# shadygm/Lichtfeld-Densification-Plugin

Hardware: AMD Instinct MI355X
Metric: triangulated points/sec + pairs/sec, MipNeRF360 garden @fast, 1/2/4/8 GPU (higher is better)
Workload: dtype f32 (+f64 Sampson/DLT solve)

## Files before the change

### include/lfd_densify.h

```cpp
#ifndef LFD_DENSIFY_H
#define LFD_DENSIFY_H

#include <stdint.h>

#ifdef __cplusplus
extern "C" {
#endif

#define LFD_ABI_VERSION 9
#define LFD_MAX_SLOTS 16

enum lfd_status {
    LFD_OK = 0,
    LFD_ERR_INVALID = 1,
    LFD_ERR_HIP = 2,
    LFD_ERR_CAPACITY = 3,
    LFD_ERR_STATE = 4
};

typedef struct lfd_context lfd_context;

typedef struct lfd_params {
    double sampson_thresh;
    float certainty_thresh;
    float sample_cap;
    float reproj_thresh;
    float min_parallax_deg;
    int32_t no_filter;
    int32_t flags;
} lfd_params;

#define LFD_FLAG_EXACT_COLOUR 1

typedef struct lfd_batch {
    int32_t n_refs;
    int32_t k;
    int32_t H, W;
    int32_t w_match, h_match;
    int32_t warp_channels;
    int32_t reserved;
    const int32_t* ref_cam;
    const int32_t* n_slots;
    const int32_t* nbr_cam;
    const float* const* cert;
    const float* const* warp;
    const uint8_t* const* image;
    const uint8_t* const* mask_a;
    const uint8_t* const* mask_b;
    const float* axis_x;
    const float* axis_y;
    const float* fundamental;
} lfd_batch;

typedef struct lfd_points {
    float* xyz;
    float* rgb;
    float* err;
    int32_t* cell;
    uint8_t* slot;
    int64_t capacity;
} lfd_points;

int lfd_abi_version(void);
int lfd_create(int device_index, void* hip_stream, lfd_context** out);
void lfd_destroy(lfd_context* ctx);
int lfd_set_stream(lfd_context* ctx, void* hip_stream);
int lfd_reload_env(lfd_context* ctx);
int lfd_kernel_timing(lfd_context* ctx, int32_t n_launches);
int lfd_kernel_timing_read(lfd_context* ctx, float* ms, int32_t capacity, int32_t* n_out);
const char* lfd_last_error(const lfd_context* ctx);
int lfd_struct_layout(int32_t* out, int32_t capacity);
const char* lfd_struct_fields(void);

int lfd_upload_cameras(lfd_context* ctx, int32_t n, const float* K, const float* R, const float* t,
                       const float* P, const float* C, const int32_t* wh);

int lfd_prepare_batch(lfd_context* ctx, const lfd_batch* batch, const lfd_params* params);

int lfd_aggregate(lfd_context* ctx, const lfd_batch* batch, const lfd_params* params,
                  float* best_cert, uint8_t* best_slot);

int lfd_triangulate_dense(lfd_context* ctx, const lfd_batch* batch, const lfd_params* params,
                          const lfd_points* out, int64_t* ref_offsets, int32_t* seg_counts);

int lfd_triangulate_dense_ply(lfd_context* ctx, const lfd_batch* batch, const lfd_params* params, uint8_t* records, int64_t capacity,
                              int64_t* ref_offsets, int32_t* seg_counts, int32_t* cell, uint8_t* slot);

typedef struct lfd_tile_segment { int32_t offset; int32_t count; } lfd_tile_segment;
#define LFD_FLAG_TILE_SEGMENTS 2
int lfd_dense_tiles_per_ref(int32_t H, int32_t W);
int lfd_triangulate_dense_segments(lfd_context* ctx, const lfd_batch* batch, const lfd_params* params, const lfd_points* out,
                                   int64_t* ref_counts, int32_t* seg_counts, lfd_tile_segment* table);
int lfd_triangulate_dense_ply_segments(lfd_context* ctx, const lfd_batch* batch, const lfd_params* params, uint8_t* records, int64_t capacity,
                                       int64_t* ref_counts, int32_t* seg_counts, lfd_tile_segment* table);
int lfd_order_segments(lfd_context* ctx, int32_t n_refs, int32_t H, int32_t W, const lfd_tile_segment* table, const lfd_points* src,
                       const lfd_points* dst, int64_t* ref_offsets);
int lfd_pack_ply_segments(lfd_context* ctx, int32_t n_refs, int32_t H, int32_t W, const lfd_tile_segment* table, const float* xyz,
                          const float* rgb, int64_t capacity, uint8_t* out, int64_t* ref_offsets);
int lfd_pack_points3d_segments(lfd_context* ctx, int32_t n_refs, int32_t H, int32_t W, const lfd_tile_segment* table, const float* xyz,
                               const float* rgb, const float* err, int64_t capacity, uint64_t id_base, uint8_t* out, int64_t* ref_offsets);

int lfd_triangulate_indexed(lfd_context* ctx, const lfd_batch* batch, const lfd_params* params,
                            const int64_t* sel_idx, const int64_t* sel_offsets, const lfd_points* out,
                            int64_t* ref_offsets, int32_t* seg_counts, int32_t* seg_order);

int lfd_triangulate_sampled(lfd_context* ctx, const lfd_batch* batch, const lfd_params* params, int32_t M, float cap,
                            int32_t border, int32_t tiles, float s_override, const lfd_points* out, int64_t* ref_offsets,
                            int32_t* seg_counts, int32_t* seg_order, int32_t* sel_info, int64_t* sel_cells);

int lfd_triangulate_sampled_multi(lfd_context* ctx, const lfd_batch* batch, const lfd_params* params, int32_t M, float cap,
                                  int32_t border, int32_t tiles, const uint32_t* seeds, const lfd_points* out,
                                  int64_t* ref_offsets, int32_t* seg_counts, int32_t* seg_order, int32_t* sel_info,
                                  int64_t* sel_cells);

int lfd_triangulate_sampled_chain(lfd_context* ctx, const lfd_batch* batch, const lfd_params* params, int32_t M, float cap,
                                  int32_t border, int32_t tiles, const float* s_overrides, const lfd_points* out,
                                  int64_t* ref_offsets, int32_t* seg_counts, int32_t* seg_order, int32_t* sel_info,
                                  int64_t* sel_cells);

int lfd_rng_seed(lfd_context* ctx, uint32_t seed);
int lfd_rng_get_state(lfd_context* ctx, uint32_t* key624_host, int32_t* pos_host);
int lfd_rng_set_state(lfd_context* ctx, const uint32_t* key624_host, int32_t pos);
#define LFD_RNG_CHECKPOINTS 4
int lfd_rng_checkpoint(lfd_context* ctx, int32_t place);
int lfd_rng_rollback(lfd_context* ctx, int32_t place);
int lfd_select_samples(lfd_context* ctx, const float* best_cert, int32_t H, int32_t W, int32_t M, float cap,
                       int32_t border, int32_t tiles, float s_override, int64_t* sel_out, int64_t capacity,
                       int32_t* n_sel_host, int32_t* status_host);

int lfd_select_top_m(lfd_context* ctx, const float* best_cert, int32_t H, int32_t W, int32_t M, float cap,
                     int64_t* sel_out, int64_t capacity, int32_t* n_sel_host, int32_t* status_host);

int lfd_pack_ply(lfd_context* ctx, const float* xyz, const float* rgb, int64_t n, uint8_t* out);
int lfd_pack_ply_normals(lfd_context* ctx, const float* xyz, const float* normals, const float* rgb, int64_t n, uint8_t* out);
int lfd_pack_points3d(lfd_context* ctx, const float* xyz, const float* rgb, const float* err, int64_t n,
                      uint64_t id_base, uint8_t* out);
int lfd_quantise_rgb(lfd_context* ctx, const float* rgb, int64_t n, uint8_t* out);

int lfd_voxel_downsample(lfd_context* ctx, const float* xyz, const float* rgb, int64_t n, double voxel_size,
                         float* xyz_out, float* rgb_out, int64_t* n_out_host);

int lfd_local_corr(lfd_context* ctx, const float* A, const float* Bf, const float* warp, int32_t B, int32_t N, int32_t C, int32_t K,
                   int32_t H1, int32_t W1, const int64_t* a_strides, const int64_t* bf_strides, float* out);
int lfd_local_corr_host(lfd_context* ctx, const float* A, const float* Bf, const float* warp, int32_t B, int32_t N, int32_t C, int32_t K,
                        int32_t H1, int32_t W1, const int64_t* a_strides, const int64_t* bf_strides, float* out);

int lfd_refiner_block(lfd_context* ctx, const void* x, int32_t x_is_f32, int32_t B, int32_t C, int32_t H, int32_t W,
                      const float* dw_w, const float* scale, const float* shift, const float* pw_wT, const float* pw_b, uint16_t* out);
int lfd_refiner_block_host(lfd_context* ctx, const void* x, int32_t x_is_f32, int32_t B, int32_t C, int32_t H, int32_t W,
                           const float* dw_w, const float* scale, const float* shift, const float* pw_wT, const float* pw_b, uint16_t* out);

int lfd_refiner_head(lfd_context* ctx, const void* z, int32_t z_is_f32, int32_t B, int32_t C, int32_t H, int32_t W, const float* head_w,
                     const float* head_b, const float* prev_warp, const int64_t* prev_warp_strides, const float* prev_conf,
                     const int64_t* prev_conf_strides, int32_t prev_dim, float refine_init, float* warp, float* conf);
int lfd_refiner_head_host(lfd_context* ctx, const void* z, int32_t z_is_f32, int32_t B, int32_t C, int32_t H, int32_t W, const float* head_w,
                          const float* head_b, const float* prev_warp, const int64_t* prev_warp_strides, const float* prev_conf,
                          const int64_t* prev_conf_strides, int32_t prev_dim, float refine_init, float* warp, float* conf);

int lfd_cycle_gate(lfd_context* ctx, int32_t n_pairs, const float* const* cert, const float* const* warp_ab, const float* const* warp_ba, int32_t H,
                   int32_t W, int32_t warp_channels, int32_t Hb, int32_t Wb, const float* axis_x, const float* axis_y, int32_t w_match,
                   int32_t h_match, float certainty_thresh, float cycle_thresh_px, float* const* cert_out, float* const* err_out,
                   int32_t* rejected);
int lfd_cycle_gate_host(lfd_context* ctx, int32_t n_pairs, const float* const* cert, const float* const* warp_ab, const float* const* warp_ba,
                        int32_t H, int32_t W, int32_t warp_channels, int32_t Hb, int32_t Wb, const float* axis_x, const float* axis_y,
                        int32_t w_match, int32_t h_match, float certainty_thresh, float cycle_thresh_px, float* const* cert_out,
                        float* const* err_out, int32_t* rejected);

// ... 171 lines not shown
```

### lichtfeld-densification-plugin_amd/core/hip_backend.py

```python
from __future__ import annotations

import ctypes as C
import threading
import dataclasses
import os
from typing import List, Optional, Sequence, Tuple

import numpy as np
import torch

from .types import CameraRecord, DensePipelineConfig

LFD_MAX_SLOTS = 16
LFD_ABI_VERSION = 9
LFD_CONSENSUS_CAP = 8
LFD_FLAG_EXACT_COLOUR = 1
LFD_FLAG_TILE_SEGMENTS = 2
_LIB_NAME = "liblfd_densify.so"
_PKG_DIR = os.path.dirname(os.path.dirname(os.path.abspath(__file__)))


class HipBackendError(RuntimeError):
    """Raised for any non-zero status of the HIP library (message from ``lfd_last_error``)."""

# ... 53 lines not shown
    _fields_ = [("xyz", C.c_void_p), ("rgb", C.c_void_p), ("err", C.c_void_p), ("cell", C.c_void_p),
                ("slot", C.c_void_p), ("capacity", C.c_int64)]


class lfd_tile_segment(C.Structure):
    _fields_ = [("offset", C.c_int32), ("count", C.c_int32)]


class lfd_copy_segment(C.Structure):
    _fields_ = [("src_offset", C.c_int64), ("dst_offset", C.c_int64), ("nbytes", C.c_int64)]


ABI_STRUCTS = (lfd_params, lfd_batch, lfd_points, lfd_tile_segment, lfd_copy_segment)


def check_struct_layout(lib, structs=ABI_STRUCTS) -> None:
    lib.lfd_struct_layout.argtypes = [C.POINTER(C.c_int32), C.c_int32]
    lib.lfd_struct_layout.restype = C.c_int
    n = int(lib.lfd_struct_layout(None, 0))
    table = (C.c_int32 * n)()
    lib.lfd_struct_layout(table, n)
    lib.lfd_struct_fields.restype = C.c_char_p
    names = dict(part.split(":") for part in lib.lfd_struct_fields().decode().split(";"))
    vals, at = list(table), 0
    for cls in structs:
        theirs = names.get(cls.__name__, "").split(",")
        if [name for name, *_ in cls._fields_] != theirs:
            raise HipBackendError(f"ctypes mirror of {cls.__name__} lists the fields {[name for name, *_ in cls._fields_]}, the library's header has "
                                  f"{theirs} (include/lfd_densify.h and core/hip_backend.py disagree)")
        if at + 2 > len(vals):
            raise HipBackendError(f"lfd_struct_layout ends before {cls.__name__}: the library is older than this binding")
        size, n_fields = vals[at], vals[at + 1]
        offsets = list(zip(vals[at + 2:at + 2 + 2 * n_fields:2], vals[at + 3:at + 2 + 2 * n_fields:2]))
        at += 2 + 2 * n_fields
        mine = [(name, getattr(cls, name).offset, getattr(cls, name).size) for name, *_ in cls._fields_]
        if C.sizeof(cls) != size or [(o, z) for _n, o, z in mine] != offsets:
            raise HipBackendError(f"ctypes mirror of {cls.__name__} does not match the library's layout: here sizeof {C.sizeof(cls)} with offsets "
                                  f"(name, offset, size) {mine}, the library has sizeof {size} with (offset, size) {offsets} (include/lfd_densify.h and core/hip_backend.py disagree)")
    if at != len(vals):
        raise HipBackendError("lfd_struct_layout reports structures this binding does not mirror")


_lib = None


def library_path() -> str:
    return os.environ.get("LFD_DENSIFY_LIB") or os.path.join(_PKG_DIR, _LIB_NAME)


def load_library() -> C.CDLL:
    global _lib
    if _lib is not None:
        return _lib
    path = library_path()
    if not os.path.exists(path):
        raise HipBackendError(
            f"{path} not found: build it with `python {os.path.join(_PKG_DIR, 'csrc', 'build.py')}` "
            "(hipcc, --offload-arch=gfx950). There is no CPU fallback for the dense-initialisation path.")
    lib = C.CDLL(path)
    ctxp = C.c_void_p
    lib.lfd_abi_version.restype = C.c_int
    if int(lib.lfd_abi_version()) != LFD_ABI_VERSION:
        raise HipBackendError(f"{path} implements ABI {int(lib.lfd_abi_version())}, this binding ABI {LFD_ABI_VERSION}: rebuild the library "
                              f"(python {os.path.join(_PKG_DIR, 'csrc', 'build.py')})")
    check_struct_layout(lib)
    lib.lfd_create.argtypes = [C.c_int, C.c_void_p, C.POINTER(ctxp)]
    lib.lfd_destroy.argtypes = [ctxp]
    lib.lfd_destroy.restype = None
    lib.lfd_set_stream.argtypes = [ctxp, C.c_void_p]
    lib.lfd_reload_env.argtypes = [ctxp]
    lib.lfd_kernel_timing.argtypes = [ctxp, C.c_int32]
    lib.lfd_kernel_timing_read.argtypes = [ctxp, C.POINTER(C.c_float), C.c_int32, C.POINTER(C.c_int32)]
    lib.lfd_last_error.argtypes = [ctxp]
    lib.lfd_last_error.restype = C.c_char_p
    fptr = C.POINTER(C.c_float)
    lib.lfd_upload_cameras.argtypes = [ctxp, C.c_int32, fptr, fptr, fptr, fptr, fptr, C.POINTER(C.c_int32)]
    lib.lfd_prepare_batch.argtypes = [ctxp, C.POINTER(lfd_batch), C.POINTER(lfd_params)]
    lib.lfd_aggregate.argtypes = [ctxp, C.POINTER(lfd_batch), C.POINTER(lfd_params), C.c_void_p, C.c_void_p]
    lib.lfd_triangulate_dense.argtypes = [ctxp, C.POINTER(lfd_batch), C.POINTER(lfd_params), C.POINTER(lfd_points),
                                          C.c_void_p, C.c_void_p]
    lib.lfd_triangulate_dense_ply.argtypes = [ctxp, C.POINTER(lfd_batch), C.POINTER(lfd_params), C.c_void_p, C.c_int64, C.c_void_p, C.c_void_p,
                                              C.c_void_p, C.c_void_p]
    lib.lfd_dense_tiles_per_ref.argtypes = [C.c_int32, C.c_int32]
    lib.lfd_triangulate_dense_segments.argtypes = [ctxp, C.POINTER(lfd_batch), C.POINTER(lfd_params), C.POINTER(lfd_points),
                                                   C.c_void_p, C.c_void_p, C.c_void_p]
    lib.lfd_triangulate_dense_ply_segments.argtypes = [ctxp, C.POINTER(lfd_batch), C.POINTER(lfd_params), C.c_void_p, C.c_int64, C.c_void_p, C.c_void_p, C.c_void_p]
    lib.lfd_order_segments.argtypes = [ctxp, C.c_int32, C.c_int32, C.c_int32, C.c_void_p, C.POINTER(lfd_points), C.POINTER(lfd_points), C.c_void_p]
    lib.lfd_pack_ply_segments.argtypes = [ctxp, C.c_int32, C.c_int32, C.c_int32, C.c_void_p, C.c_void_p, C.c_void_p, C.c_int64, C.c_void_p, C.c_void_p]
    lib.lfd_pack_points3d_segments.argtypes = [ctxp, C.c_int32, C.c_int32, C.c_int32, C.c_void_p, C.c_void_p, C.c_void_p, C.c_void_p, C.c_int64,
                                               C.c_uint64, C.c_void_p, C.c_void_p]
    lib.lfd_triangulate_indexed.argtypes = [ctxp, C.POINTER(lfd_batch), C.POINTER(lfd_params), C.c_void_p,
                                            C.POINTER(C.c_int64), C.POINTER(lfd_points), C.c_void_p, C.c_void_p,
                                            C.c_void_p]
    lib.lfd_triangulate_sampled.argtypes = [ctxp, C.POINTER(lfd_batch), C.POINTER(lfd_params), C.c_int32, C.c_float, C.c_int32,
                                            C.c_int32, C.c_float, C.POINTER(lfd_points), C.c_void_p, C.c_void_p, C.c_void_p,
                                            C.c_void_p, C.c_void_p]
    lib.lfd_triangulate_sampled_multi.argtypes = [ctxp, C.POINTER(lfd_batch), C.POINTER(lfd_params), C.c_int32, C.c_float, C.c_int32,
                                                  C.c_int32, C.POINTER(C.c_uint32), C.POINTER(lfd_points), C.c_void_p, C.c_void_p, C.c_void_p,
                                                  C.c_void_p, C.c_void_p]
    lib.lfd_triangulate_sampled_chain.argtypes = [ctxp, C.POINTER(lfd_batch), C.POINTER(lfd_params), C.c_int32, C.c_float, C.c_int32,
                                                  C.c_int32, C.POINTER(C.c_float), C.POINTER(lfd_points), C.c_void_p, C.c_void_p, C.c_void_p,
                                                  C.c_void_p, C.c_void_p]
    lib.lfd_select_top_m.argtypes = [ctxp, C.c_void_p, C.c_int32, C.c_int32, C.c_int32, C.c_float, C.c_void_p, C.c_int64,
                                     C.POINTER(C.c_int32), C.POINTER(C.c_int32)]
    lib.lfd_pack_ply.argtypes = [ctxp, C.c_void_p, C.c_void_p, C.c_int64, C.c_void_p]
    lib.lfd_pack_points3d.argtypes = [ctxp, C.c_void_p, C.c_void_p, C.c_void_p, C.c_int64, C.c_uint64, C.c_void_p]
    lib.lfd_voxel_downsample.argtypes = [ctxp, C.c_void_p, C.c_void_p, C.c_int64, C.c_double, C.c_void_p, C.c_void_p, C.POINTER(C.c_int64)]
    lib.lfd_quantise_rgb.argtypes = [ctxp, C.c_void_p, C.c_int64, C.c_void_p]
    lib.lfd_local_corr.argtypes = [ctxp, C.c_void_p, C.c_void_p, C.c_void_p] + [C.c_int32] * 6 + [C.POINTER(C.c_int64), C.POINTER(C.c_int64), C.c_void_p]
    lib.lfd_local_corr_host.argtypes = list(lib.lfd_local_corr.argtypes)
    lib.lfd_refiner_block.argtypes = [ctxp, C.c_void_p] + [C.c_int32] * 5 + [C.c_void_p] * 6
    lib.lfd_refiner_block_host.argtypes = list(lib.lfd_refiner_block.argtypes)
    lib.lfd_refiner_head.argtypes = ([ctxp, C.c_void_p] + [C.c_int32] * 5 + [C.c_void_p, C.c_void_p, C.c_void_p, C.POINTER(C.c_int64), C.c_void_p,
                                     C.POINTER(C.c_int64), C.c_int32, C.c_float, C.c_void_p, C.c_void_p])
    lib.lfd_refiner_head_host.argtypes = list(lib.lfd_refiner_head.argtypes)
    lib.lfd_cycle_gate.argtypes = ([ctxp, C.c_int32, C.c_void_p, C.c_void_p, C.c_void_p] + [C.c_int32] * 5 + [C.c_void_p, C.c_void_p, C.c_int32, C.c_int32,
                                   C.c_float, C.c_float, C.c_void_p, C.c_void_p, C.c_void_p])
    lib.lfd_cycle_gate_host.argtypes = list(lib.lfd_cycle_gate.argtypes)
    lib.lfd_support_filter.argtypes = [ctxp, C.POINTER(lfd_batch), C.POINTER(lfd_points), C.c_void_p, C.c_int32, C.c_float, C.POINTER(lfd_points),
                                       C.c_void_p, C.c_void_p, C.c_void_p]
    lib.lfd_support_filter_host.argtypes = list(lib.lfd_support_filter.argtypes)
    lib.lfd_refine_multiview.argtypes = [ctxp, C.POINTER(lfd_batch), C.POINTER(lfd_points), C.c_void_p, C.c_float, C.c_float, C.c_void_p, C.c_void_p,
                                         C.c_void_p, C.c_void_p]
    lib.lfd_refine_multiview_host.argtypes = list(lib.lfd_refine_multiview.argtypes)
    lib.lfd_refine_multiview_weighted.argtypes = list(lib.lfd_refine_multiview.argtypes) + [C.c_void_p]
    lib.lfd_refine_multiview_weighted_host.argtypes = list(lib.lfd_refine_multiview_weighted.argtypes)
    lib.lfd_depth_sigma_filter.argtypes = [ctxp, C.POINTER(lfd_batch), C.POINTER(lfd_points), C.c_void_p, C.c_void_p, C.c_float, C.c_void_p, C.c_float,
                                           C.c_float, C.POINTER(lfd_points), C.c_void_p, C.c_void_p, C.c_void_p, C.c_void_p]
    lib.lfd_depth_sigma_filter_host.argtypes = list(lib.lfd_depth_sigma_filter.argtypes)
    lib.lfd_estimate_normals.argtypes = [ctxp, C.POINTER(lfd_batch), C.POINTER(lfd_points), C.c_void_p, C.c_int32, C.c_float, C.c_float, C.c_void_p,
                                         C.c_void_p, C.c_void_p]
    lib.lfd_estimate_normals_host.argtypes = list(lib.lfd_estimate_normals.argtypes)
    lib.lfd_colour_multiview.argtypes = [ctxp, C.POINTER(lfd_batch), C.POINTER(lfd_points), C.c_void_p, C.c_void_p, C.c_float, C.c_int32, C.c_void_p,
                                         C.c_void_p, C.c_void_p]
    lib.lfd_colour_multiview_host.argtypes = list(lib.lfd_colour_multiview.argtypes)
    lib.lfd_photo_gate.argtypes = [ctxp, C.POINTER(lfd_batch), C.POINTER(lfd_points), C.c_void_p, C.c_void_p, C.c_int32, C.c_float, C.c_float,
                                   C.POINTER(lfd_points), C.c_void_p, C.c_void_p, C.c_void_p, C.c_void_p, C.c_void_p]
    lib.lfd_photo_gate_host.argtypes = list(lib.lfd_photo_gate.argtypes)
    lib.lfd_gain_accumulate.argtypes = [ctxp, C.POINTER(lfd_batch), C.POINTER(lfd_points), C.c_void_p, C.c_void_p, C.c_float, C.c_void_p]
    lib.lfd_gain_accumulate_host.argtypes = list(lib.lfd_gain_accumulate.argtypes)
    lib.lfd_gain_apply.argtypes = [ctxp, C.c_void_p, C.c_int64, C.c_void_p, C.c_int32, C.c_void_p, C.c_void_p]
    lib.lfd_gain_apply_host.argtypes = list(lib.lfd_gain_apply.argtypes)
    lib.lfd_far_accumulate.argtypes = [ctxp, C.POINTER(lfd_batch), C.c_float, C.c_float, C.c_int32, C.c_int32, C.c_void_p, C.c_void_p]
    lib.lfd_far_accumulate_host.argtypes = list(lib.lfd_far_accumulate.argtypes)
    lib.lfd_far_accumulate_flags.argtypes = list(lib.lfd_far_accumulate.argtypes) + [C.c_void_p]
    lib.lfd_far_accumulate_flags_host.argtypes = list(lib.lfd_far_accumulate_flags.argtypes)
    lib.lfd_epipolar_audit.argtypes = [ctxp, C.POINTER(lfd_batch), C.c_float, C.c_void_p, C.c_void_p]
    lib.lfd_epipolar_audit_host.argtypes = list(lib.lfd_epipolar_audit.argtypes)
    lib.lfd_pose_accumulate.argtypes = [ctxp, C.POINTER(lfd_batch), C.c_float, C.c_float, C.c_void_p]
    lib.lfd_pose_accumulate_host.argtypes = list(lib.lfd_pose_accumulate.argtypes)
    lib.lfd_far_emit.argtypes = [ctxp, C.c_void_p, C.c_int32, C.c_int64, C.POINTER(C.c_double), C.c_double, C.c_void_p, C.c_void_p, C.c_void_p,
                                 C.c_void_p, C.c_int64, C.POINTER(C.c_int64)]
    lib.lfd_far_emit_host.argtypes = list(lib.lfd_far_emit.argtypes)
    lib.lfd_pack_ply_normals.argtypes = [ctxp, C.c_void_p, C.c_void_p, C.c_void_p, C.c_int64, C.c_void_p]
    lib.lfd_consensus_filter.argtypes = [ctxp, C.c_void_p, C.c_void_p, C.c_void_p, C.c_int64, C.POINTER(C.c_int64), C.c_int32, C.c_float, C.c_int32,
                                         C.c_void_p, C.c_void_p, C.c_void_p, C.POINTER(C.c_int64), C.c_void_p, C.POINTER(C.c_int64)]
    lib.lfd_consensus_filter_host.argtypes = list(lib.lfd_consensus_filter.argtypes)
    lib.lfd_freespace_filter.argtypes = [ctxp, C.c_void_p, C.c_void_p, C.c_void_p, C.c_int64, C.POINTER(C.c_int64), C.c_int32, C.POINTER(C.c_float),
                                         C.POINTER(C.c_int32), C.c_int32, C.c_int32, C.c_float, C.c_int32, C.c_void_p, C.c_void_p, C.c_void_p,
                                         C.POINTER(C.c_int64), C.c_void_p, C.c_void_p, C.POINTER(C.c_int64)]
    lib.lfd_freespace_filter_host.argtypes = list(lib.lfd_freespace_filter.argtypes)
    lib.lfd_render_depth.argtypes = [ctxp, C.c_void_p, C.c_int64, C.c_void_p, C.POINTER(C.c_float), C.POINTER(C.c_int32), C.c_int32, C.c_int32, C.c_int32,
                                     C.c_int32, C.c_int32, C.c_float, C.c_int32, C.c_void_p, C.c_void_p, C.c_void_p]
    lib.lfd_render_depth_host.argtypes = list(lib.lfd_render_depth.argtypes)
    lib.lfd_fuse_oriented.argtypes = [ctxp, C.c_void_p, C.c_void_p, C.c_void_p, C.c_int64, C.c_double, C.c_void_p, C.c_void_p, C.c_void_p, C.c_void_p,
                                      C.POINTER(C.c_int64), C.POINTER(C.c_int64)]
    lib.lfd_fuse_oriented_host.argtypes = list(lib.lfd_fuse_oriented.argtypes)
    lib.lfd_knn_dist2.argtypes = [ctxp, C.c_void_p, C.c_int64, C.c_double, C.c_void_p, C.POINTER(C.c_double)]
    lib.lfd_knn_dist2_host.argtypes = list(lib.lfd_knn_dist2.argtypes)
    lib.lfd_pack_gaussians.argtypes = [ctxp, C.c_void_p, C.c_void_p, C.c_void_p, C.c_void_p, C.c_int64, C.c_float, C.c_double, C.c_double, C.c_void_p]
    lib.lfd_pack_gaussians_host.argtypes = list(lib.lfd_pack_gaussians.argtypes)
    lib.lfd_cap_spatial.argtypes = [ctxp, C.c_void_p, C.c_void_p, C.c_int64, C.c_int64, C.c_void_p, C.POINTER(C.c_int64), C.POINTER(C.c_double)]
    lib.lfd_cap_spatial_host.argtypes = list(lib.lfd_cap_spatial.argtypes)
    lib.lfd_thin_footprint.argtypes = [ctxp, C.c_void_p, C.c_void_p, C.c_int64, C.POINTER(C.c_int64), C.c_int32, C.POINTER(C.c_double), C.c_double,
                                       C.c_void_p, C.POINTER(C.c_int64), C.POINTER(C.c_int64), C.POINTER(C.c_double)]
    lib.lfd_thin_footprint_host.argtypes = list(lib.lfd_thin_footprint.argtypes)
    lib.lfd_copy_segments.argtypes = [C.c_void_p, C.c_int32, C.c_void_p, C.c_void_p, C.c_void_p, C.c_int32]
    lib.lfd_launch_status.argtypes = [ctxp, C.POINTER(C.c_int32)]
    lib.lfd_get_pair_fundamental.argtypes = [ctxp, C.c_int32, C.POINTER(C.c_double)]
    lib.lfd_rng_seed.argtypes = [ctxp, C.c_uint32]
    lib.lfd_rng_get_state.argtypes = [ctxp, C.POINTER(C.c_uint32), C.POINTER(C.c_int32)]
    lib.lfd_rng_set_state.argtypes = [ctxp, C.POINTER(C.c_uint32), C.c_int32]
    lib.lfd_rng_checkpoint.argtypes = [ctxp, C.c_int32]
    lib.lfd_rng_rollback.argtypes = [ctxp, C.c_int32]
    lib.lfd_select_samples.argtypes = [ctxp, C.c_void_p, C.c_int32, C.c_int32, C.c_int32, C.c_float, C.c_int32, C.c_int32,
                                       C.c_float, C.c_void_p, C.c_int64, C.POINTER(C.c_int32), C.POINTER(C.c_int32)]
    lib.lfd_create_host.argtypes = [C.c_int32, C.POINTER(ctxp)]
    lib.lfd_host_threads.argtypes = [ctxp]
    lib.lfd_host_threads.restype = C.c_int
    lib.lfd_aggregate_host.argtypes = [ctxp, C.POINTER(lfd_batch), C.POINTER(lfd_params), C.c_void_p, C.c_void_p]
    lib.lfd_triangulate_dense_host.argtypes = [ctxp, C.POINTER(lfd_batch), C.POINTER(lfd_params), C.POINTER(lfd_points),
                                               C.c_void_p, C.c_void_p]
    lib.lfd_triangulate_indexed_host.argtypes = [ctxp, C.POINTER(lfd_batch), C.POINTER(lfd_params), C.c_void_p,
                                                 C.POINTER(C.c_int64), C.POINTER(lfd_points), C.c_void_p, C.c_void_p, C.c_void_p]
    lib.lfd_prepare_image.argtypes = [ctxp, C.c_void_p, C.c_int32, C.c_int32, C.c_int32, C.c_int32, C.c_void_p, C.c_void_p]
    lib.lfd_prepare_mask.argtypes = [ctxp, C.c_void_p, C.c_int32, C.c_int32, C.c_int32, C.c_int32, C.c_float, C.c_int32, C.c_void_p]
    dptr = C.POINTER(C.c_double)
    lib.lfd_undistort_image.argtypes = [ctxp, C.c_void_p, C.c_int32, C.c_int32, C.c_int32, C.c_int32, dptr, dptr, C.c_void_p, C.c_void_p, C.POINTER(C.c_int64)]
    lib.lfd_host_undistort_image.argtypes = list(lib.lfd_undistort_image.argtypes[1:])
    lib.lfd_host_resize_tables.argtypes = [C.c_int32, C.c_int32, C.POINTER(C.c_int32), C.POINTER(C.c_int32), C.c_int32, C.POINTER(C.c_int32)]
    lib.lfd_host_nearest_indices.argtypes = [C.c_int32, C.c_int32, C.POINTER(C.c_int32)]
    lib.lfd_identity_axis.argtypes = [C.c_int32, fptr]
    lib.lfd_parallax_dot_threshold.argtypes = [C.c_float]
    lib.lfd_parallax_dot_threshold.restype = C.c_float
    lib.lfd_host_fundamental.argtypes = [fptr] * 7
    lib.lfd_host_null_vector.argtypes = [fptr, C.POINTER(C.c_double)]
    lib.lfd_host_null_vector.restype = C.c_int
    lib.lfd_host_null_vector_sym.argtypes = [C.POINTER(C.c_double), C.POINTER(C.c_double)]
    lib.lfd_host_null_vector_sym.restype = C.c_int
    lib.lfd_host_eval_correspondence.argtypes = [fptr, fptr, C.c_float, C.c_float, C.c_float, C.c_float, C.c_int32,
                                                 C.c_int32, C.POINTER(lfd_params), fptr]
    for name in ("lfd_create", "lfd_set_stream", "lfd_reload_env", "lfd_kernel_timing", "lfd_kernel_timing_read", "lfd_upload_cameras", "lfd_prepare_batch", "lfd_aggregate", "lfd_triangulate_dense",
                 "lfd_triangulate_dense_ply", "lfd_triangulate_dense_ply_segments", "lfd_dense_tiles_per_ref", "lfd_triangulate_dense_segments", "lfd_order_segments", "lfd_pack_ply_segments", "lfd_pack_points3d_segments",
                 "lfd_triangulate_indexed", "lfd_triangulate_sampled", "lfd_triangulate_sampled_multi", "lfd_triangulate_sampled_chain", "lfd_launch_status", "lfd_rng_seed", "lfd_rng_get_state", "lfd_rng_set_state",
                 "lfd_rng_checkpoint", "lfd_rng_rollback",
                 "lfd_select_samples", "lfd_select_top_m", "lfd_pack_ply", "lfd_pack_points3d", "lfd_voxel_downsample", "lfd_local_corr", "lfd_local_corr_host", "lfd_refiner_block", "lfd_refiner_block_host", "lfd_refiner_head", "lfd_refiner_head_host", "lfd_cycle_gate", "lfd_cycle_gate_host", "lfd_support_filter", "lfd_support_filter_host", "lfd_refine_multiview", "lfd_refine_multiview_host", "lfd_refine_multiview_weighted", "lfd_refine_multiview_weighted_host", "lfd_depth_sigma_filter", "lfd_depth_sigma_filter_host", "lfd_estimate_normals", "lfd_estimate_normals_host", "lfd_colour_multiview", "lfd_photo_gate", "lfd_photo_gate_host", "lfd_colour_multiview_host", "lfd_gain_accumulate", "lfd_gain_accumulate_host", "lfd_gain_apply", "lfd_gain_apply_host", "lfd_far_accumulate", "lfd_far_accumulate_host", "lfd_far_accumulate_flags", "lfd_far_accumulate_flags_host", "lfd_far_emit", "lfd_far_emit_host", "lfd_pack_ply_normals", "lfd_consensus_filter", "lfd_consensus_filter_host", "lfd_freespace_filter", "lfd_freespace_filter_host", "lfd_render_depth", "lfd_render_depth_host", "lfd_fuse_oriented", "lfd_fuse_oriented_host", "lfd_knn_dist2", "lfd_knn_dist2_host", "lfd_pack_gaussians", "lfd_pack_gaussians_host", "lfd_cap_spatial", "lfd_cap_spatial_host", "lfd_thin_footprint", "lfd_thin_footprint_host", "lfd_quantise_rgb", "lfd_copy_segments", "lfd_identity_axis",
                 "lfd_host_fundamental", "lfd_get_pair_fundamental", "lfd_create_host", "lfd_aggregate_host",
                 "lfd_triangulate_dense_host", "lfd_triangulate_indexed_host", "lfd_prepare_image", "lfd_prepare_mask",
                 "lfd_host_resize_tables", "lfd_host_nearest_indices",
                 "lfd_host_eval_correspondence"):
        getattr(lib, name).restype = C.c_int
    _lib = lib
    return lib


def make_params(config: DensePipelineConfig, sample_cap: float = 0.9, exact_colour: Optional[bool] = None) -> lfd_params:
    if exact_colour is None:
        exact_colour = bool(config.exact_colour)
    floor = float(config.certainty_thresh)
    if float(config.exp("cycle_thresh_px")) > 0.0:
        floor = min(floor, 0.0)
    return lfd_params(sampson_thresh=float(config.sampson_thresh), certainty_thresh=floor,
                      sample_cap=float(sample_cap), reproj_thresh=float(config.reproj_thresh),
                      min_parallax_deg=float(config.min_parallax_deg), no_filter=1 if config.no_filter else 0,
                      flags=LFD_FLAG_EXACT_COLOUR if exact_colour else 0)


def _f32(a) -> np.ndarray:
    return np.ascontiguousarray(np.asarray(a, np.float32))


def _fp(a: np.ndarray):
    return a.ctypes.data_as(C.POINTER(C.c_float))


def identity_axis(n: int) -> np.ndarray:
    out = np.empty(n, np.float32)
    rc = load_library().lfd_identity_axis(n, _fp(out))
    if rc != 0:
        raise HipBackendError("lfd_identity_axis failed")
    return out


def copy_segments(src: torch.Tensor, dst: torch.Tensor, segments, stream: Optional["torch.cuda.Stream"] = None) -> None:
    segs = np.ascontiguousarray(np.asarray(segments, np.int64).reshape(-1, 3))
    if segs.shape[0] == 0:
        return
    if not (src.is_cuda and dst.is_cuda and src.device == dst.device and src.is_contiguous() and dst.is_contiguous()):
        raise ValueError("copy_segments needs two contiguous tensors on one GPU")
    sb, db = src.numel() * src.element_size(), dst.numel() * dst.element_size()
    if segs.min() < 0 or int((segs[:, 0] + segs[:, 2]).max()) > sb or int((segs[:, 1] + segs[:, 2]).max()) > db:
        raise ValueError("copy_segments: a segment leaves its tensor")
    st = stream if stream is not None else torch.cuda.current_stream(src.device)
    rc = load_library().lfd_copy_segments(C.c_void_p(st.cuda_stream), int(src.device.index or 0), C.c_void_p(src.data_ptr()), C.c_void_p(dst.data_ptr()),
                                          segs.ctypes.data_as(C.c_void_p), int(segs.shape[0]))
    if rc != 0:
        raise HipBackendError(f"lfd_copy_segments failed ({rc})")


def parallax_dot_threshold(min_deg: float) -> float:
    return float(load_library().lfd_parallax_dot_threshold(C.c_float(min_deg)))


def host_fundamental(K1, R1, t1, K2, R2, t2) -> np.ndarray:
    a = [_f32(x).reshape(-1) for x in (K1, R1, t1, K2, R2, t2)]
    out = np.empty(9, np.float32)
    rc = load_library().lfd_host_fundamental(*[_fp(x) for x in a], _fp(out))
    if rc != 0:
        raise HipBackendError("lfd_host_fundamental failed")
    return out.reshape(3, 3)


def host_resize_tables(in_size: int, out_size: int):
    lib = load_library()
    ks = C.c_int32(0)
    bounds = np.zeros((out_size, 2), np.int32)
    kk = np.zeros((1,), np.int32)
    lib.lfd_host_resize_tables(in_size, out_size, bounds.ctypes.data_as(C.POINTER(C.c_int32)), kk.ctypes.data_as(C.POINTER(C.c_int32)), 0, C.byref(ks))
    kk = np.zeros((out_size, int(ks.value)), np.int32)
    rc = lib.lfd_host_resize_tables(in_size, out_size, bounds.ctypes.data_as(C.POINTER(C.c_int32)), kk.ctypes.data_as(C.POINTER(C.c_int32)),
                                    int(kk.size), C.byref(ks))
    if rc != 0:
        raise HipBackendError("lfd_host_resize_tables failed")
    return bounds, kk


def host_nearest_indices(in_size: int, out_size: int) -> np.ndarray:
    idx = np.zeros((out_size,), np.int32)
    if load_library().lfd_host_nearest_indices(in_size, out_size, idx.ctypes.data_as(C.POINTER(C.c_int32))) != 0:
        raise HipBackendError("lfd_host_nearest_indices failed")
    return idx


def _undistort_parameters(distortion):
    d = [float(v) for v in distortion]
    if len(d) != 12:
        raise ValueError("distortion must hold twelve values: fx, fy, cx, cy, k1, k2, p1, p2, k3, k4, k5, k6")
    return (C.c_double * 4)(*d[:4]), (C.c_double * 8)(*d[4:])


def host_undistort_image(src, distortion, nearest: bool = False, with_valid: bool = False):
    a = np.ascontiguousarray(src, dtype=np.uint8)
    if a.ndim not in (2, 3) or (a.ndim == 3 and a.shape[2] != 3):
        raise ValueError("src must be a (h, w) or (h, w, 3) uint8 array")
    h, w = int(a.shape[0]), int(a.shape[1])
    intr, dist = _undistort_parameters(distortion)
    dst = np.empty_like(a)
    valid = np.empty((h, w), np.uint8) if with_valid else None
    n_bad = C.c_int64(-1)
    rc = load_library().lfd_host_undistort_image(a.ctypes.data, w, h, 1 if a.ndim == 2 else 3, 1 if nearest else 0, intr, dist, dst.ctypes.data,
# ... 1926 lines not shown
```

### lichtfeld-densification-plugin_amd/csrc/lfd_api.hip

```cpp
#include <cstddef>
#include <hip/hip_runtime.h>
#include <hip/hip_ext.h>

#include <algorithm>
#include <cmath>
#include <cstdio>
#include <cstdlib>
#include <cstring>
#include <mutex>
#include <string>
#include <vector>

#include "lfd_context.hpp"
#include "lfd_corr.hpp"
#include "lfd_block.hpp"
#include "lfd_head.hpp"
#include "lfd_cycle.hpp"
#include "lfd_support.hpp"
#include "lfd_refine.hpp"
#include "lfd_normals.hpp"
#include "lfd_colour.hpp"
#include "lfd_photo.hpp"
#include "lfd_gain.hpp"
#include "lfd_far.hpp"
#include "lfd_audit.hpp"
#include "lfd_pose.hpp"
#include "lfd_sigma.hpp"
#include "lfd_consensus.hpp"
#include "lfd_undistort.hpp"
#include "lfd_freespace.hpp"
#include "lfd_depth.hpp"
#include "lfd_fuse.hpp"
#include "lfd_knn.hpp"
#include "lfd_cap.hpp"
#include "lfd_thin.hpp"

extern "C" __global__ void lfd_aggregate_kernel(LfdLaunch L, float* best_cert, uint8_t* best_slot);
extern "C" __global__ void lfd_dense_kernel(LfdLaunch L);
extern "C" __global__ void lfd_dense_exact_kernel(LfdLaunch L);
extern "C" __global__ void lfd_dense_ply_kernel(LfdLaunch L);
extern "C" __global__ void lfd_dense_ply_exact_kernel(LfdLaunch L);
extern "C" __global__ void lfd_dense_segments_kernel(LfdLaunch L);
extern "C" __global__ void lfd_dense_segments_exact_kernel(LfdLaunch L);
extern "C" __global__ void lfd_dense_ply_segments_kernel(LfdLaunch L);
extern "C" __global__ void lfd_dense_ply_segments_exact_kernel(LfdLaunch L);
extern "C" __global__ void lfd_segment_scan_kernel(const LfdTileSeg* table, int n_tiles, int tiles_per_ref, int n_refs, long long* tile_dst, long long* ref_offsets);
extern "C" __global__ void lfd_order_segments_kernel(const long long* tile_dst, const LfdTileSeg* table, long long hw, int tiles_per_ref, int n_tiles,
                                                     const float* sxyz, const float* srgb, const float* serr, const int* scell, const unsigned char* sslot,
                                                     float* dxyz, float* drgb, float* derr, int* dcell, unsigned char* dslot, long long capacity);
extern "C" __global__ void lfd_pack_ply_segments_kernel(const long long* tile_dst, const LfdTileSeg* table, long long hw, int tiles_per_ref, int n_tiles,
                                                        const float* xyz, const float* rgb, long long capacity, unsigned char* out);
extern "C" __global__ void lfd_pack_points3d_segments_kernel(const long long* tile_dst, const LfdTileSeg* table, long long hw, int tiles_per_ref, int n_tiles,
                                                             const float* xyz, const float* rgb, const float* err, long long capacity,
                                                             unsigned long long id_base, unsigned char* out);
extern "C" __global__ void lfd_pair_setup_kernel(LfdLaunch L, LfdRefConst* ref_out, LfdPairConst* pair_out);
extern "C" __global__ void lfd_select_filter_kernel(LfdSelectArgs A);
extern "C" __global__ void lfd_pack_ply_kernel(const float* xyz, const float* rgb, long long n, unsigned char* out);
extern "C" __global__ void lfd_pack_points3d_kernel(const float* xyz, const float* rgb, const float* err, long long n,
                                                    unsigned long long id_base, unsigned char* out);
extern "C" __global__ void lfd_copy_segments_kernel(LfdCopyArgs A, const unsigned char* src, unsigned char* dst);
extern "C" __global__ void lfd_quantise_rgb_kernel(const float* rgb, long long n3, unsigned char* out);
extern "C" __global__ void lfd_voxel_minmax_kernel(const float* xyz, const float* rgb, long long n, LfdVoxStats* part);
extern "C" __global__ void lfd_voxel_final_kernel(const LfdVoxStats* part, int n_part, LfdVoxStats* out);
extern "C" __global__ void lfd_voxel_keys_kernel(const float* xyz, long long n, double o0, double o1, double o2, double vs, unsigned long long e1,
                                                 unsigned long long e2, unsigned long long* keys, unsigned* idx);
extern "C" __global__ void lfd_voxel_hist_kernel(const unsigned long long* keys, long long n, long long chunk, int shift, unsigned* counts);
extern "C" __global__ void lfd_voxel_scan_kernel(unsigned* v, int m, unsigned* total);
extern "C" __global__ void lfd_voxel_scatter_kernel(const unsigned long long* kin, const unsigned* iin, long long n, long long chunk, int shift,
                                                    const unsigned* counts, unsigned long long* kout, unsigned* iout);
extern "C" __global__ void lfd_voxel_head_count_kernel(const unsigned long long* keys, long long n, long long chunk, unsigned* counts);
extern "C" __global__ void lfd_voxel_head_scatter_kernel(const unsigned long long* keys, long long n, long long chunk, const unsigned* counts,
                                                         unsigned* vstart);
extern "C" __global__ void lfd_voxel_sums_kernel(const float* xyz, const float* rgb, long long n, const unsigned* sorted_idx, const unsigned* vstart,
                                                 const unsigned* nv_p, double cscale, float* xyz_out, float* rgb_out, unsigned* big, unsigned* n_big);
extern "C" __global__ void lfd_voxel_sums_big_kernel(const float* xyz, const float* rgb, long long n, const unsigned* sorted_idx, const unsigned* vstart,
                                                     const unsigned* nv_p, double cscale, const unsigned* big, const unsigned* n_big, float* xyz_out,
                                                     float* rgb_out);
hipError_t lfd_undistort_launch(const LfdUndistortArgs& p, unsigned long long* n_invalid, hipStream_t stream);
extern "C" __global__ void lfd_consensus_minmax_kernel(const float* xyz, long long n, LfdVoxStats* part);
extern "C" __global__ void lfd_consensus_keys_kernel(const float* xyz, long long n, double o0, double o1, double o2, double h, unsigned long long e1,
                                                     unsigned long long e2, unsigned long long sentinel, unsigned long long* keys, unsigned* idx);
extern "C" __global__ void lfd_consensus_gather_kernel(const float* xyz, const unsigned* sorted_idx, const long long* offs, int n_refs, long long n,
                                                       LfdConsensusPt* spt);
extern "C" __global__ void lfd_consensus_count_kernel(const unsigned long long* skey, const LfdConsensusPt* spt, const unsigned* sorted_idx, long long n,
                                                      unsigned long long e1, unsigned long long e2, unsigned long long sentinel, float r2, int min_refs,
                                                      int bound, uint8_t* keep, uint8_t* consensus);
extern "C" __global__ void lfd_consensus_wgcount_kernel(const uint8_t* keep, long long n, unsigned* wg_kept);
extern "C" __global__ void lfd_consensus_offsets_kernel(const long long* offs, int n_refs, const uint8_t* keep, const unsigned* wg_kept, long long* offs_out);
extern "C" __global__ void lfd_consensus_scatter_kernel(const float* xyz, const float* rgb, const float* err, long long n, const uint8_t* keep,
                                                        const unsigned* wg_kept, float* o_xyz, float* o_rgb, float* o_err);
extern "C" __global__ void lfd_fuse_side_kernel(const float* normals, long long n, const unsigned* sorted_idx, const unsigned* vstart, const unsigned* nv_p,
                                                uint8_t* flag, unsigned* rows, unsigned* big, unsigned* n_big);
extern "C" __global__ void lfd_fuse_side_big_kernel(const float* normals, long long n, const unsigned* sorted_idx, const unsigned* vstart, const unsigned* nv_p,
                                                    const unsigned* big, const unsigned* n_big, uint8_t* flag, unsigned* rows);
extern "C" __global__ void lfd_fuse_rowsum_kernel(const unsigned* rows, const unsigned* nv_p, long long chunk, unsigned* counts);
extern "C" __global__ void lfd_fuse_rowstart_kernel(unsigned* rows, const unsigned* nv_p, long long chunk, const unsigned* counts);
extern "C" __global__ void lfd_fuse_sums_kernel(const float* xyz, const float* normals, const float* rgb, long long n, const unsigned* sorted_idx,
                                                const unsigned* vstart, const unsigned* nv_p, const uint8_t* flag, const unsigned* rowstart, double cscale,
                                                float* xyz_out, float* normals_out, float* rgb_out, unsigned* count_out);
extern "C" __global__ void lfd_fuse_sums_big_kernel(const float* xyz, const float* normals, const float* rgb, long long n, const unsigned* sorted_idx,
                                                    const unsigned* vstart, const unsigned* nv_p, const uint8_t* flag, const unsigned* rowstart, double cscale,
                                                    const unsigned* big, const unsigned* n_big, float* xyz_out, float* normals_out, float* rgb_out,
                                                    unsigned* count_out);
extern "C" __global__ void lfd_knn_keys_kernel(const float* xyz, long long n, LfdKnnGrid g, unsigned long long* keys, unsigned* idx);
extern "C" __global__ void lfd_knn_cellmax_kernel(const unsigned* vstart, const unsigned* nv_p, long long n, unsigned* max_out);
extern "C" __global__ void lfd_knn_gather_kernel(const float* xyz, const unsigned* sorted_idx, long long n, LfdKnnPt* spt);
extern "C" __global__ void lfd_knn_scan_kernel(const unsigned long long* skey, const LfdKnnPt* spt, long long n, LfdKnnGrid g, float* dist2, unsigned* list,
                                               unsigned* n_list);
extern "C" __global__ void lfd_knn_brute_kernel(const LfdKnnPt* spt, long long n, const unsigned* list, const unsigned* n_list, float* dist2);
extern "C" __global__ void lfd_pack_gaussians_kernel(const float* xyz, const float* normals, const float* rgb, const float* dist2, long long n, float opacity,
                                                     double log_flatten, float max_m, float* out);
extern "C" __global__ void lfd_cap_keys_kernel(const float* xyz, long long n, LfdCapBox box, unsigned long long* keys, unsigned* idx);
extern "C" __global__ void lfd_cap_levels_kernel(const unsigned long long* keys, long long n, unsigned* hist);
extern "C" __global__ void lfd_cap_coarsen_kernel(unsigned long long* keys, long long n, int shift);
extern "C" __global__ void lfd_cap_rep_kernel(const unsigned* sorted_idx, const unsigned* vstart, const unsigned* nc_p, const float* err, long long n,
                                              unsigned long long budget, unsigned long long* rep);
extern "C" __global__ void lfd_cap_mark_kernel(const unsigned long long* rep, const unsigned* nc_p, long long n, unsigned long long budget, uint8_t* keep);
extern "C" __global__ void lfd_cap_index_kernel(const uint8_t* keep, const unsigned* wg_kept, long long n, long long capacity, long long* keep_out);
extern "C" __global__ void lfd_thin_keys_kernel(const float* xyz, long long n, const long long* offs, int n_refs, const double* rows, double thin_cells,
                                                LfdCapBox box, unsigned long long* keys, unsigned* idx, unsigned* hist);
extern "C" __global__ void lfd_thin_cells_kernel(const unsigned long long* keys, const unsigned* vstart, const unsigned* nc_p, long long n, unsigned* hist);
extern "C" __global__ void lfd_freespace_fill_kernel(uint32_t* zbuf, long long n_words);
// ... 20 lines not shown
hipError_t lfd_gain_launch(const LfdGainArgs& p, hipStream_t stream);
hipError_t lfd_gain_apply_launch(const LfdGainApplyArgs& p, hipStream_t stream);
hipError_t lfd_far_launch(const LfdFarArgs& p, bool reduce, hipStream_t stream);
hipError_t lfd_far_mark_launch(const unsigned long long* table, long long n_cells, long long min_samples, uint8_t* keep, hipStream_t stream);
hipError_t lfd_far_emit_launch(const LfdFarEmitArgs& p, hipStream_t stream);
hipError_t lfd_audit_launch(const LfdAuditArgs& p, bool aggregate, hipStream_t stream);
hipError_t lfd_pose_launch(const LfdPoseArgs& p, hipStream_t stream);
extern "C" __global__ void lfd_pack_ply_normals_kernel(const float* xyz, const float* normals, const float* rgb, long long n, unsigned char* out);
extern "C" __global__ void lfd_select_topm_kernel(LfdSelectArgs A);
extern "C" __global__ void lfd_select_filter_mw_kernel(LfdSelectArgs A, LfdSelectNorms norms);
extern "C" __global__ void lfd_select_begins_kernel(long long* pairs, long long stride, int n);
extern "C" __global__ void lfd_mt_seed_kernel(unsigned* mt, unsigned seed);
extern "C" __global__ void lfd_mt_seed_batch_kernel(unsigned* mt_base, LfdSeedBatch seeds);
extern "C" __global__ void lfd_indexed_eval_kernel(LfdLaunch L, const long long* sel_idx, const long long* sel_offsets, float* scratch,
                                                   uint8_t* codes, unsigned* tab, int off_pairs);
extern "C" __global__ void lfd_indexed_kernel(LfdLaunch L, const long long* sel_idx, const long long* sel_offsets,
                                              float* scratch, uint8_t* codes, int32_t* seg_order, const unsigned* tab, int off_pairs);

namespace {

std::mutex g_create_mutex;
std::string g_create_error;
thread_local std::string t_create_error_copy;

}

namespace {

int fail(lfd_context* ctx, int code, const std::string& msg) { return lfd_fail(ctx, code, msg); }

#define LFD_HIP(ctx, expr)                                                                         \
    do {                                                                                           \
        hipError_t e_ = (expr);                                                                    \
        if (e_ != hipSuccess)                                                                      \
            return fail((ctx), LFD_ERR_HIP, std::string(#expr) + ": " + hipGetErrorString(e_));    \
    } while (0)

int ensure(lfd_context* ctx, DeviceBuffer& b, size_t bytes, bool zero = false) {
    if (b.bytes >= bytes && b.ptr) return LFD_OK;
    if (b.ptr) {
        LFD_HIP(ctx, hipStreamSynchronize(ctx->stream));
        if (ctx->prep_stream) LFD_HIP(ctx, hipStreamSynchronize(ctx->prep_stream));
        LFD_HIP(ctx, hipFree(b.ptr));
        b.ptr = nullptr; b.bytes = 0;
    }
    size_t want = std::max<size_t>(bytes, 256);
    want = (want + 255) & ~size_t(255);
    LFD_HIP(ctx, hipMalloc(&b.ptr, want));
    b.bytes = want;
    if (zero) LFD_HIP(ctx, hipMemsetAsync(b.ptr, 0, want, ctx->stream));
    return LFD_OK;
}

int validate_batch(lfd_context* ctx, const lfd_batch* b, const lfd_params* p) {
    if (!ctx) return fail(nullptr, LFD_ERR_INVALID, "null context");
    if (ctx->is_host) return fail(ctx, LFD_ERR_STATE, "this context was made by lfd_create_host: it serves the *_host entry points only");
    if (!b || !p) return fail(ctx, LFD_ERR_INVALID, "null batch/params");
    if (ctx->n_cams <= 0) return fail(ctx, LFD_ERR_STATE, "lfd_upload_cameras must be called first");
    if (b->n_refs <= 0) return fail(ctx, LFD_ERR_INVALID, "n_refs must be > 0");
    if (b->k <= 0 || b->k > LFD_MAX_SLOTS) return fail(ctx, LFD_ERR_INVALID, "k must be in [1, LFD_MAX_SLOTS]");
    if (b->H <= 0 || b->W <= 0 || b->w_match <= 1 || b->h_match <= 1) return fail(ctx, LFD_ERR_INVALID, "bad grid / match size");
    if (b->w_match >= (1 << 24) || b->h_match >= (1 << 24) || (long long)b->w_match * b->h_match * 3 > 0x7fffffffLL)
        return fail(ctx, LFD_ERR_INVALID, "match-size image too large");
    if ((long long)b->H * b->W > 0x7fffffffLL) return fail(ctx, LFD_ERR_INVALID, "grid too large");
    if (b->warp_channels != 2 && b->warp_channels != 4) return fail(ctx, LFD_ERR_INVALID, "warp_channels must be 2 or 4");
    if (!b->ref_cam || !b->n_slots || !b->nbr_cam || !b->cert || !b->warp || !b->image)
        return fail(ctx, LFD_ERR_INVALID, "null table in batch");
    if ((b->axis_x == nullptr) != (b->axis_y == nullptr)) return fail(ctx, LFD_ERR_INVALID, "axis_x and axis_y must both be given or both be null");
    for (int r = 0; r < b->n_refs; ++r) {
        if (b->ref_cam[r] < 0 || b->ref_cam[r] >= ctx->n_cams) return fail(ctx, LFD_ERR_INVALID, "ref_cam out of range");
        if (b->n_slots[r] < 1 || b->n_slots[r] > b->k) return fail(ctx, LFD_ERR_INVALID, "n_slots must be in [1, k]");
        if (!b->image[r]) return fail(ctx, LFD_ERR_INVALID, "null image pointer");
        for (int j = 0; j < b->n_slots[r]; ++j) {
            const size_t s = (size_t)r * b->k + j;
            if (b->nbr_cam[s] < 0 || b->nbr_cam[s] >= ctx->n_cams) return fail(ctx, LFD_ERR_INVALID, "nbr_cam out of range");
            if (!b->cert[s] || !b->warp[s]) return fail(ctx, LFD_ERR_INVALID, "null cert/warp pointer in a valid slot");
            if ((reinterpret_cast<uintptr_t>(b->cert[s]) & 15u) || (reinterpret_cast<uintptr_t>(b->warp[s]) & 15u))
                return fail(ctx, LFD_ERR_INVALID, "cert/warp planes must be 16-byte aligned");
        }
    }
    return LFD_OK;
}

int slot_events(lfd_context* ctx, LfdBatchSlot& sl) {
    if (!sl.pinned_free) LFD_HIP(ctx, hipEventCreateWithFlags(&sl.pinned_free, hipEventDisableTiming));
    if (!sl.ready) LFD_HIP(ctx, hipEventCreateWithFlags(&sl.ready, hipEventDisableTiming));
    if (!sl.idle) LFD_HIP(ctx, hipEventCreateWithFlags(&sl.idle, hipEventDisableTiming));
    return LFD_OK;
}

int upload_tables(lfd_context* ctx, const lfd_batch* b, const long long* extra, size_t n_extra, bool ahead, int* slot_out, hipStream_t* stream_out,
                  const LfdRefDesc** d_refs, const LfdSlotDesc** d_slots, const long long** d_extra, const float** d_fund) {
    const size_t nr = (size_t)b->n_refs, ns = nr * (size_t)b->k;
    const size_t off_slots = (nr * sizeof(LfdRefDesc) + 15) & ~size_t(15);
    const size_t off_fund = (off_slots + ns * sizeof(LfdSlotDesc) + 15) & ~size_t(15);
    const size_t total = (off_fund + (b->fundamental ? ns * 9 * sizeof(float) : 0) + 15) & ~size_t(15);
    const size_t off_extra = total;
    const size_t extra_room = ((nr + 1) * sizeof(long long) + 15) & ~size_t(15);
    std::vector<unsigned char> blob(total, 0);
    LfdRefDesc* refs = reinterpret_cast<LfdRefDesc*>(blob.data());
    LfdSlotDesc* slots = reinterpret_cast<LfdSlotDesc*>(blob.data() + off_slots);
    for (size_t r = 0; r < nr; ++r) {
        refs[r].image = b->image[r];
        refs[r].mask_a = b->mask_a ? b->mask_a[r] : nullptr;
        refs[r].cam = b->ref_cam[r];
        refs[r].n_slots = b->n_slots[r];
        refs[r].any_mask = refs[r].mask_a ? 1 : 0;
        refs[r].pad = 0;
        for (int j = 0; j < b->k; ++j) {
            LfdSlotDesc& s = slots[r * b->k + j];
            const bool valid = j < b->n_slots[r];
            s.cert = valid ? b->cert[r * b->k + j] : nullptr;
            s.warp = valid ? b->warp[r * b->k + j] : nullptr;
            s.mask_b = (valid && b->mask_b) ? b->mask_b[r * b->k + j] : nullptr;
            s.cam = valid ? b->nbr_cam[r * b->k + j] : 0;
            s.pad = 0;
            if (s.mask_b) refs[r].any_mask = 1;
        }
    }
    if (b->fundamental) std::memcpy(blob.data() + off_fund, b->fundamental, ns * 9 * sizeof(float));
    if (n_extra * sizeof(long long) > extra_room) return fail(ctx, LFD_ERR_INVALID, "internal: selection offsets beyond the reserved room");

    int si = -1;
    for (int c = 0; c < 2; ++c) {
        const int i = c == 0 ? ctx->cur : 1 - ctx->cur;
        if (ctx->slot[i].desc.ptr && ctx->slot[i].cache == blob) { si = i; break; }
    }
    hipStream_t st = ctx->stream;
    if (si >= 0) {
        LfdBatchSlot& sl = ctx->slot[si];
        if (!ahead && sl.ready_pending) {
#if !defined(LFD_EXPERIMENT_NO_READY_WAIT)
            LFD_HIP(ctx, hipStreamWaitEvent(ctx->stream, sl.ready, 0));
#endif
            sl.ready_pending = false;
        }
        if (ahead && sl.ready_pending) st = ctx->prep_stream;
    } else {
        if (ahead) {
            if (!ctx->prep_stream) LFD_HIP(ctx, hipStreamCreateWithFlags(&ctx->prep_stream, hipStreamNonBlocking));
            si = ctx->last_used < 0 ? ctx->cur : 1 - ctx->cur;
            st = ctx->prep_stream;
        } else {
            si = ctx->cur;
        }
        LfdBatchSlot& sl = ctx->slot[si];
        int rc = slot_events(ctx, sl);
        if (rc != LFD_OK) return rc;
        if (ahead) {
            if (sl.used) LFD_HIP(ctx, hipStreamWaitEvent(st, sl.idle_attached ? sl.idle_ext : sl.idle, 0));
        } else if (sl.ready_pending) {
            LFD_HIP(ctx, hipStreamWaitEvent(ctx->stream, sl.ready, 0));
            sl.ready_pending = false;
        }
        rc = ensure(ctx, sl.desc, total + extra_room);
        if (rc != LFD_OK) return rc;
        if (sl.pinned_bytes < total + extra_room) {
            if (sl.pinned_in_flight) { LFD_HIP(ctx, hipEventSynchronize(sl.pinned_free)); sl.pinned_in_flight = false; }
            if (sl.pinned) LFD_HIP(ctx, hipHostFree(sl.pinned));
            sl.pinned = nullptr;
            sl.pinned_bytes = std::max<size_t>((total + extra_room) * 2, 1 << 16);
            LFD_HIP(ctx, hipHostMalloc(&sl.pinned, sl.pinned_bytes, hipHostMallocDefault));
        }
        if (sl.pinned_in_flight) { LFD_HIP(ctx, hipEventSynchronize(sl.pinned_free)); sl.pinned_in_flight = false; }
        std::memcpy(sl.pinned, blob.data(), total);
        LFD_HIP(ctx, hipMemcpyAsync(sl.desc.ptr, sl.pinned, total, hipMemcpyHostToDevice, st));
        LFD_HIP(ctx, hipEventRecord(sl.pinned_free, st));
        sl.pinned_in_flight = true;
        sl.cache.swap(blob);
        sl.consts_valid = false;
    }
    LfdBatchSlot& sl = ctx->slot[si];
    if (n_extra) {
        if (sl.desc.bytes < total + extra_room) return fail(ctx, LFD_ERR_STATE, "internal: batch slot without room for the selection offsets");
        if (sl.x_in_flight) { LFD_HIP(ctx, hipEventSynchronize(sl.x_free)); sl.x_in_flight = false; }
        if (sl.pinned_x_bytes < extra_room) {
            if (sl.pinned_x) LFD_HIP(ctx, hipHostFree(sl.pinned_x));
            sl.pinned_x = nullptr;
            sl.pinned_x_bytes = std::max<size_t>(extra_room * 2, 4096);
            LFD_HIP(ctx, hipHostMalloc(&sl.pinned_x, sl.pinned_x_bytes, hipHostMallocDefault));
        }
        if (!sl.x_free) LFD_HIP(ctx, hipEventCreateWithFlags(&sl.x_free, hipEventDisableTiming));
        std::memcpy(sl.pinned_x, extra, n_extra * sizeof(long long));
        LFD_HIP(ctx, hipMemcpyAsync(static_cast<unsigned char*>(sl.desc.ptr) + off_extra, sl.pinned_x, n_extra * sizeof(long long), hipMemcpyHostToDevice,
                                    ctx->stream));
        LFD_HIP(ctx, hipEventRecord(sl.x_free, ctx->stream));
        sl.x_in_flight = true;
    }
    *slot_out = si;
    *stream_out = st;
    *d_refs = reinterpret_cast<const LfdRefDesc*>(sl.desc.ptr);
    *d_slots = reinterpret_cast<const LfdSlotDesc*>(static_cast<unsigned char*>(sl.desc.ptr) + off_slots);
    if (d_extra) *d_extra = reinterpret_cast<const long long*>(static_cast<unsigned char*>(sl.desc.ptr) + off_extra);
    *d_fund = b->fundamental ? reinterpret_cast<const float*>(static_cast<unsigned char*>(sl.desc.ptr) + off_fund) : nullptr;
    return LFD_OK;
}

int default_axes(lfd_context* ctx, int W, int H, const float** ax, const float** ay) {
    if (ctx->axes_w != W || ctx->axes_h != H || !ctx->axes.ptr) {
        int rc = ensure(ctx, ctx->axes, sizeof(float) * (size_t)(W + H));
        if (rc != LFD_OK) return rc;
        std::vector<float> host((size_t)W + H);
        lfd_identity_axis(W, host.data());
        lfd_identity_axis(H, host.data() + W);
        LFD_HIP(ctx, hipMemcpyAsync(ctx->axes.ptr, host.data(), host.size() * sizeof(float), hipMemcpyHostToDevice, ctx->stream));
        LFD_HIP(ctx, hipStreamSynchronize(ctx->stream));
        ctx->axes_w = W; ctx->axes_h = H;
    }
    *ax = static_cast<const float*>(ctx->axes.ptr);
    *ay = *ax + W;
    return LFD_OK;
}

int colour_tables(lfd_context* ctx, int W, int H, int wm, int hm, const LfdColourCol** cols, const LfdColourRow** rows) {
    const int key[4] = {W, H, wm, hm};
    if (!ctx->colour_tab.ptr || std::memcmp(key, ctx->colour_key, sizeof(key)) != 0) {
        static_assert(sizeof(LfdColourCol) == 16 && sizeof(LfdColourRow) == 16, "colour table entries are 16 bytes");
        int rc = ensure(ctx, ctx->colour_tab, sizeof(LfdColourCol) * (size_t)W + sizeof(LfdColourRow) * (size_t)H);
        if (rc != LFD_OK) return rc;
        std::vector<unsigned char> host(sizeof(LfdColourCol) * (size_t)W + sizeof(LfdColourRow) * (size_t)H);
        LfdColourCol* hc = reinterpret_cast<LfdColourCol*>(host.data());
        LfdColourRow* hr = reinterpret_cast<LfdColourRow*>(host.data() + sizeof(LfdColourCol) * (size_t)W);
        const LfdAxis ax = lfd_make_axis(W), ay = lfd_make_axis(H);
        for (int x = 0; x < W; ++x) hc[x] = lfd_colour_col(lfd_match_px(lfd_axis_value(ax, x), (float)(wm - 1)), wm);
        for (int y = 0; y < H; ++y) hr[y] = lfd_colour_row(lfd_match_px(lfd_axis_value(ay, y), (float)(hm - 1)), wm, hm);
        LFD_HIP(ctx, hipMemcpyAsync(ctx->colour_tab.ptr, host.data(), host.size(), hipMemcpyHostToDevice, ctx->stream));
        LFD_HIP(ctx, hipStreamSynchronize(ctx->stream));
        std::memcpy(ctx->colour_key, key, sizeof(key));
    }
    *cols = static_cast<const LfdColourCol*>(ctx->colour_tab.ptr);
    *rows = reinterpret_cast<const LfdColourRow*>(static_cast<const unsigned char*>(ctx->colour_tab.ptr) + sizeof(LfdColourCol) * (size_t)W);
    return LFD_OK;
}

}

void lfd_fill_kernel_params(const lfd_batch* b, const lfd_params* p, LfdKernelParams& kp) {
    kp.sampson_thresh = p->sampson_thresh;
    kp.certainty_thresh = p->certainty_thresh;
    kp.reproj_thresh = p->reproj_thresh;
    kp.no_filter = p->no_filter ? 1 : 0;
    (void)LFD_FLAG_EXACT_COLOUR;
    kp.use_sampson = (!p->no_filter && p->sampson_thresh > 0.0) ? 1 : 0;
    kp.use_parallax = (!p->no_filter && p->min_parallax_deg > 0.0f) ? 1 : 0;
    kp.dot_thresh = kp.use_parallax ? lfd_parallax_dot_threshold(p->min_parallax_deg) : 2.0f;
    kp.wm1 = (float)(b->w_match - 1);
    kp.hm1 = (float)(b->h_match - 1);
}

namespace {

int prepare_launch(lfd_context* ctx, const lfd_batch* b, const lfd_params* p, const long long* extra, size_t n_extra,
                   LfdLaunch& L, const long long** d_extra, bool ahead = false) {
    int rc = validate_batch(ctx, b, p);
    if (rc != LFD_OK) return rc;
    LFD_HIP(ctx, hipSetDevice(ctx->device));
    std::memset(&L, 0, sizeof(L));
    if (!ahead && ctx->last_used >= 0) {
        LfdBatchSlot& prev = ctx->slot[ctx->last_used];
        rc = slot_events(ctx, prev);
        if (rc != LFD_OK) return rc;
        if (!prev.idle_attached) LFD_HIP(ctx, hipEventRecord(prev.idle, ctx->stream));
        prev.used = true;
    }
    int si = 0;
// ... 10 lines not shown
    }
    L.ax = lfd_make_axis(b->W);
    L.ay = lfd_make_axis(b->H);
    L.n_refs = b->n_refs; L.k = b->k; L.H = b->H; L.W = b->W;
    L.w_match = b->w_match; L.h_match = b->h_match; L.warp_channels = b->warp_channels;
    const long long HW = (long long)b->H * b->W;
    const int tile = LFD_DENSE_BLOCK * LFD_DENSE_CPT;
    L.tiles_per_ref = (int)((HW + tile - 1) / tile);
    L.mask_sx = (float)b->w_match / (float)b->W;
    L.mask_sy = (float)b->h_match / (float)b->H;
    L.inv_w = 1.0f / (float)b->W;
    L.w_log2 = -1;
    if ((b->W & (b->W - 1)) == 0) { int l = 0; while ((1 << l) < b->W) ++l; L.w_log2 = l; }
    lfd_fill_kernel_params(b, p, L.kp);
    const size_t ref_bytes = ((size_t)b->n_refs * sizeof(LfdRefConst) + 15) & ~size_t(15);
    const size_t need = ref_bytes + (size_t)b->n_refs * b->k * sizeof(LfdPairConst);
    if (sl.consts.bytes < need) sl.consts_valid = false;
    rc = ensure(ctx, sl.consts, need);
    if (rc != LFD_OK) return rc;
    LfdRefConst* d_rc = static_cast<LfdRefConst*>(sl.consts.ptr);
    LfdPairConst* d_pc = reinterpret_cast<LfdPairConst*>(static_cast<unsigned char*>(sl.consts.ptr) + ref_bytes);
    L.ref_const = d_rc;
    L.pair_const = d_pc;
    if (!sl.consts_valid || sl.wm != b->w_match || sl.hm != b->h_match) {
        const int n = b->n_refs * b->k + b->n_refs;
        hipLaunchKernelGGL(lfd_pair_setup_kernel, dim3((unsigned)((n + 63) / 64)), dim3(64), 0, st, L, d_rc, d_pc);
        LFD_HIP(ctx, hipGetLastError());
        sl.consts_valid = true;
        sl.refs = b->n_refs; sl.k = b->k;
        sl.wm = b->w_match;
        sl.hm = b->h_match;
        if (st != ctx->stream) {
            LFD_HIP(ctx, hipEventRecord(sl.ready, st));
            sl.ready_pending = true;
        }
    }
    if (!ahead) {
        ctx->cur = si; ctx->last_used = si;
        sl.idle_attached = false;
    }
    return LFD_OK;
}

constexpr size_t kWsHeader = 128 + 128 * LFD_TICKET_LANES;

int prepare_lookback(lfd_context* ctx, size_t n_tiles, size_t n_tickets, bool lanes, LfdLaunch& L) {
    const size_t need = kWsHeader + n_tiles * sizeof(unsigned long long);
    const bool fresh = ctx->ws.bytes < need || !ctx->ws.ptr;
    int rc = ensure(ctx, ctx->ws, need, true);
    if (rc != LFD_OK) return rc;
    if (fresh) {
        ctx->tickets_issued = 0; ctx->epoch = 0;
        for (int s = 0; s < LFD_TICKET_LANES; ++s) ctx->lane_issued[s] = 0;
    }
    ctx->epoch = (ctx->epoch + 1) & LFD_EPOCH_MASK;
    if (ctx->epoch == 0) {
        LFD_HIP(ctx, hipMemsetAsync(static_cast<unsigned char*>(ctx->ws.ptr) + kWsHeader, 0, ctx->ws.bytes - kWsHeader, ctx->stream));
        LFD_HIP(ctx, hipMemsetAsync(static_cast<unsigned char*>(ctx->ws.ptr) + 16, 0, 4, ctx->stream));
        ctx->epoch = 1;
    }
    unsigned char* base = static_cast<unsigned char*>(ctx->ws.ptr);
    L.ticket = reinterpret_cast<unsigned long long*>(base);
    L.ticket_lanes = reinterpret_cast<unsigned long long*>(base + 128);
    L.tile_state = reinterpret_cast<unsigned long long*>(base + kWsHeader);
    L.status = reinterpret_cast<unsigned int*>(base + 8);
    L.seg_ready = reinterpret_cast<unsigned int*>(base + 16);
    L.ticket_base = ctx->tickets_issued;
    L.epoch = ctx->epoch;
    if (lanes) {
        for (int s = 0; s < LFD_TICKET_LANES; ++s) {
            L.ticket_base_lane[s] = ctx->lane_issued[s];
            if ((size_t)s < n_tickets) ctx->lane_issued[s] += (n_tickets - (size_t)s + LFD_TICKET_LANES - 1) / LFD_TICKET_LANES;
        }
    } else {
        ctx->tickets_issued += n_tickets;
    }
    return LFD_OK;
}

void read_env_switches(lfd_context* ctx) {
    ctx->env = LfdEnvSwitches();
    if (const char* e = std::getenv("LFD_DENSE_EXTRA_LDS")) ctx->env.dense_extra_lds = (size_t)std::atol(e);
    if (const char* e = std::getenv("LFD_DENSE_TIMING")) ctx->env.dense_timing_path = e;
    if (const char* e = std::getenv("LFD_INDEXED_SPLIT")) ctx->env.indexed_split = std::atoi(e) != 0;
    if (const char* e = std::getenv("LFD_SELECT_TIMING")) ctx->env.select_timing = std::max(1, std::atoi(e));
    if (const char* e = std::getenv("LFD_SELECT_WORKGROUPS")) ctx->env.select_workgroups = std::atoi(e);
}

int check_points(lfd_context* ctx, const lfd_points* out, const long long* ref_offsets) {
    if (!out || !out->xyz || !out->rgb || !out->err) return fail(ctx, LFD_ERR_INVALID, "null output buffers");
    if (out->capacity < 0) return fail(ctx, LFD_ERR_INVALID, "negative capacity");
    if (!ref_offsets) return fail(ctx, LFD_ERR_INVALID, "ref_offsets is required");
    return LFD_OK;
}

int batch_launch(lfd_context* ctx, const lfd_batch* batch, LfdLaunch& L) {
    lfd_params none;
    std::memset(&none, 0, sizeof(none));
    return prepare_launch(ctx, batch, &none, nullptr, 0, L, nullptr);
}

struct CloudPlan {
    long long n;
    long long G, chunk;
    int n_part;
    long long n_wg;
    unsigned grid;
};

CloudPlan cloud_plan(int64_t n) {
    CloudPlan p;
    p.n = n;
    p.G = std::min<long long>(1024, (n + 4095) / 4096);
    p.chunk = (((n + p.G - 1) / p.G) + 511) / 512 * 512;
    p.G = (n + p.chunk - 1) / p.chunk;
    p.n_part = (int)std::min<long long>(1024, (n + 255) / 256);
    p.n_wg = (n + 255) / 256;
    p.grid = (unsigned)std::min<long long>(p.n_wg, 4096);
    return p;
}

struct Bump {
    unsigned char* base;
    size_t at = 0;
    template <class T>
    T* take(size_t count, size_t extra_bytes = 0) {
        const size_t o = at;
        at = (at + count * sizeof(T) + extra_bytes + 255) & ~size_t(255);
        return base ? reinterpret_cast<T*>(base + o) : nullptr;
    }
};

template <class Layout>
int carve_cloud_ws(lfd_context* ctx, Layout&& layout) {
    Bump size{nullptr};
    layout(size);
    if (int rc = ensure(ctx, ctx->cloud_ws, size.at)) return rc;
    Bump b{static_cast<unsigned char*>(ctx->cloud_ws.ptr)};
    layout(b);
    return LFD_OK;
}

struct CloudSort {
    LfdVoxStats *part, *stats;
    unsigned* counters;
    unsigned* counts;
    unsigned long long* keys[2];
    unsigned* idx[2];
    unsigned* vstart;
};

CloudSort carve_sort(Bump& b, long long n, int n_counters, bool heads) {
    CloudSort w;
    w.part = b.take<LfdVoxStats>(1024);
    w.stats = b.take<LfdVoxStats>(1, (size_t)n_counters * sizeof(unsigned));
    w.counters = w.stats ? reinterpret_cast<unsigned*>(w.stats + 1) : nullptr;
    w.counts = b.take<unsigned>(256 * 1024);
    for (int i = 0; i < 2; ++i) w.keys[i] = b.take<unsigned long long>((size_t)n);
    for (int i = 0; i < 2; ++i) w.idx[i] = b.take<unsigned>((size_t)n);
    w.vstart = heads ? b.take<unsigned>((size_t)n) : nullptr;
    return w;
}

int cloud_stats(lfd_context* ctx, const CloudPlan& p, const CloudSort& w, const float* xyz, const float* rgb, LfdVoxStats& s) {
    hipStream_t st = ctx->stream;
    if (rgb) hipLaunchKernelGGL(lfd_voxel_minmax_kernel, dim3(p.n_part), dim3(256), 0, st, xyz, rgb, p.n, w.part);
// ... 92 lines not shown
    const int32_t n = (int32_t)(sizeof(table) / sizeof(table[0]));
    for (int32_t i = 0; out != nullptr && i < n && i < capacity; ++i) out[i] = table[i];
    return n;
}

const char* lfd_struct_fields(void) {
    return "lfd_params:sampson_thresh,certainty_thresh,sample_cap,reproj_thresh,min_parallax_deg,no_filter,flags;"
           "lfd_batch:n_refs,k,H,W,w_match,h_match,warp_channels,reserved,ref_cam,n_slots,nbr_cam,cert,warp,image,mask_a,mask_b,axis_x,axis_y,fundamental;"
           "lfd_points:xyz,rgb,err,cell,slot,capacity;"
           "lfd_tile_segment:offset,count;"
           "lfd_copy_segment:src_offset,dst_offset,nbytes";
}

const char* lfd_last_error(const lfd_context* ctx) {
    if (ctx) return ctx->err.c_str();
    std::lock_guard<std::mutex> lock(g_create_mutex);
    t_create_error_copy = g_create_error;
    return t_create_error_copy.c_str();
}

int lfd_create(int device_index, void* hip_stream, lfd_context** out) {
    if (!out) return fail(nullptr, LFD_ERR_INVALID, "out is null");
    *out = nullptr;
    int n = 0;
    hipError_t e = hipGetDeviceCount(&n);
    if (e != hipSuccess || n <= 0)
        return fail(nullptr, LFD_ERR_HIP, std::string("no HIP device available: ") + (e != hipSuccess ? hipGetErrorString(e) : "device count is 0"));
    if (device_index < 0 || device_index >= n) return fail(nullptr, LFD_ERR_INVALID, "device index out of range");
    lfd_context* ctx = new lfd_context();
    ctx->device = device_index;
    ctx->stream = static_cast<hipStream_t>(hip_stream);
    read_env_switches(ctx);
    e = hipSetDevice(device_index);
    if (e == hipSuccess) e = hipDeviceGetAttribute(&ctx->n_cus, hipDeviceAttributeMultiprocessorCount, device_index);
    if (e == hipSuccess) e = hipHostMalloc(reinterpret_cast<void**>(&ctx->pinned_words), 32 * sizeof(int), hipHostMallocDefault);
    if (e != hipSuccess) {
        std::string m = std::string("context init: ") + hipGetErrorString(e);
        delete ctx;
        return fail(nullptr, LFD_ERR_HIP, m);
    }
    *out = ctx;
    return LFD_OK;
}

void lfd_destroy(lfd_context* ctx) {
    if (!ctx) return;
    if (ctx->is_host) { lfd_host_pool_destroy(ctx->host_pool); delete ctx; return; }
    (void)hipSetDevice(ctx->device);
    (void)hipStreamSynchronize(ctx->stream);
    if (ctx->prep_stream) { (void)hipStreamSynchronize(ctx->prep_stream); (void)hipStreamDestroy(ctx->prep_stream); }
    for (LfdBatchSlot& sl : ctx->slot) {
        if (sl.desc.ptr) (void)hipFree(sl.desc.ptr);
        if (sl.consts.ptr) (void)hipFree(sl.consts.ptr);
        if (sl.pinned) (void)hipHostFree(sl.pinned);
        if (sl.pinned_x) (void)hipHostFree(sl.pinned_x);
        for (hipEvent_t ev : {sl.pinned_free, sl.ready, sl.idle, sl.x_free}) if (ev) (void)hipEventDestroy(ev);
    }
    for (hipEvent_t ev : ctx->kt_start) (void)hipEventDestroy(ev);
    for (hipEvent_t ev : ctx->kt_stop) (void)hipEventDestroy(ev);
    for (DeviceBuffer* b : {&ctx->cams, &ctx->ws, &ctx->axes, &ctx->scratch, &ctx->codes, &ctx->idx_tab, &ctx->agg, &ctx->sel_buf, &ctx->colour_tab, &ctx->mt, &ctx->mt_ckpt, &ctx->mt_batch, &ctx->sel_scratch, &ctx->sel_chain, &ctx->stamps, &ctx->img_tab, &ctx->msk_tab, &ctx->seg_scan, &ctx->cloud_ws, &ctx->support_ws, &ctx->prec.tab, &ctx->colour_img.tab, &ctx->pose_const.tab, &ctx->undist_cnt})
        if (b->ptr) (void)hipFree(b->ptr);
    if (ctx->pinned_words) (void)hipHostFree(ctx->pinned_words);
    for (lfd_context::PointerTable* t : {&ctx->prec, &ctx->colour_img, &ctx->pose_const}) {
        if (t->pinned) (void)hipHostFree(t->pinned);
        if (t->free_ev) (void)hipEventDestroy(t->free_ev);
    }
    delete ctx;
}

int lfd_kernel_timing(lfd_context* ctx, int32_t n_launches) {
    if (!ctx) return fail(nullptr, LFD_ERR_INVALID, "null context");
    if (ctx->is_host) return fail(ctx, LFD_ERR_STATE, "device entry point called on a host context");
    if (n_launches < 0 || n_launches > (1 << 20)) return fail(ctx, LFD_ERR_INVALID, "lfd_kernel_timing: n_launches must be in [0, 2^20]");
    LFD_HIP(ctx, hipSetDevice(ctx->device));
    LFD_HIP(ctx, hipStreamSynchronize(ctx->stream));
    if (ctx->prep_stream) LFD_HIP(ctx, hipStreamSynchronize(ctx->prep_stream));
    for (LfdBatchSlot& sl : ctx->slot) { sl.idle_attached = false; sl.idle_ext = nullptr; sl.used = false; }
    while (ctx->kt_start.size() > (size_t)n_launches) {
        (void)hipEventDestroy(ctx->kt_start.back()); (void)hipEventDestroy(ctx->kt_stop.back());
        ctx->kt_start.pop_back(); ctx->kt_stop.pop_back();
    }
    while (ctx->kt_start.size() < (size_t)n_launches) {
        hipEvent_t a = nullptr, b = nullptr;
        LFD_HIP(ctx, hipEventCreate(&a));
        hipError_t e = hipEventCreate(&b);
        if (e != hipSuccess) { (void)hipEventDestroy(a); return fail(ctx, LFD_ERR_HIP, std::string("hipEventCreate: ") + hipGetErrorString(e)); }
        ctx->kt_start.push_back(a); ctx->kt_stop.push_back(b);
    }
    ctx->kt_used = 0;
    return LFD_OK;
}

int lfd_kernel_timing_read(lfd_context* ctx, float* ms, int32_t capacity, int32_t* n_out) {
    if (!ctx) return fail(nullptr, LFD_ERR_INVALID, "null context");
    if (ctx->is_host) return fail(ctx, LFD_ERR_STATE, "device entry point called on a host context");
    if (!n_out || capacity < 0 || (capacity > 0 && !ms)) return fail(ctx, LFD_ERR_INVALID, "lfd_kernel_timing_read: bad arguments");
    LFD_HIP(ctx, hipSetDevice(ctx->device));
    const size_t n = std::min(ctx->kt_used, (size_t)capacity);
    if (ctx->kt_used) LFD_HIP(ctx, hipEventSynchronize(ctx->kt_stop[ctx->kt_used - 1]));
    for (size_t i = 0; i < n; ++i) LFD_HIP(ctx, hipEventElapsedTime(ms + i, ctx->kt_start[i], ctx->kt_stop[i]));
    *n_out = (int32_t)n;
    ctx->kt_used = 0;
    return LFD_OK;
}

int lfd_reload_env(lfd_context* ctx) {
    if (!ctx) return fail(nullptr, LFD_ERR_INVALID, "null context");
    read_env_switches(ctx);
    return LFD_OK;
}

int lfd_set_stream(lfd_context* ctx, void* hip_stream) {
    if (!ctx) return fail(nullptr, LFD_ERR_INVALID, "null context");
    if (ctx->is_host) return fail(ctx, LFD_ERR_STATE, "device entry point called on a host context");
    LFD_HIP(ctx, hipSetDevice(ctx->device));
    LFD_HIP(ctx, hipStreamSynchronize(ctx->stream));
    if (ctx->prep_stream) LFD_HIP(ctx, hipStreamSynchronize(ctx->prep_stream));
    for (LfdBatchSlot& sl : ctx->slot) { sl.ready_pending = false; sl.used = false; sl.idle_attached = false; }
    ctx->last_used = -1;
    ctx->stream = static_cast<hipStream_t>(hip_stream);
    return LFD_OK;
}

int lfd_launch_status(lfd_context* ctx, int32_t* status_out) {
    if (!ctx || !status_out) return fail(ctx, LFD_ERR_INVALID, "null argument");
    *status_out = 0;
    if (ctx->is_host) return LFD_OK;
    LFD_HIP(ctx, hipSetDevice(ctx->device));
    if (!ctx->ws.ptr) { LFD_HIP(ctx, hipStreamSynchronize(ctx->stream)); return LFD_OK; }
    LFD_HIP(ctx, hipMemcpyAsync(ctx->pinned_words, static_cast<unsigned char*>(ctx->ws.ptr) + 8, sizeof(unsigned int), hipMemcpyDeviceToHost, ctx->stream));
    LFD_HIP(ctx, hipStreamSynchronize(ctx->stream));
    const unsigned int st = (unsigned int)ctx->pinned_words[0];
    if (st != 0) {
        LFD_HIP(ctx, hipMemset(static_cast<unsigned char*>(ctx->ws.ptr) + 8, 0, sizeof(st)));
        *status_out = (int32_t)st;
        return fail(ctx, LFD_ERR_HIP, "a look-back spin timed out (workgroups of the persistent grid were not co-resident); results of the last launch are invalid");
    }
    return LFD_OK;
}

int lfd_get_pair_fundamental(lfd_context* ctx, int32_t n_pairs, double* F_out_host) {
    if (!ctx || !F_out_host || n_pairs <= 0) return fail(ctx, LFD_ERR_INVALID, "bad arguments");
    if (ctx->is_host) return fail(ctx, LFD_ERR_STATE, "device entry point called on a host context");
    const LfdBatchSlot& sl = ctx->slot[ctx->cur];
    if (ctx->last_used < 0 || !sl.consts_valid || !sl.consts.ptr) return fail(ctx, LFD_ERR_STATE, "no batch has been launched on this context yet");
    if (n_pairs != sl.refs * sl.k) return fail(ctx, LFD_ERR_INVALID, "n_pairs must be n_refs * k of the last batch");
    LFD_HIP(ctx, hipSetDevice(ctx->device));
    const size_t ref_bytes = ((size_t)sl.refs * sizeof(LfdRefConst) + 15) & ~size_t(15);
    std::vector<LfdPairConst> host((size_t)n_pairs);
    LFD_HIP(ctx, hipMemcpyAsync(host.data(), static_cast<unsigned char*>(sl.consts.ptr) + ref_bytes, host.size() * sizeof(LfdPairConst),
                                hipMemcpyDeviceToHost, ctx->stream));
    LFD_HIP(ctx, hipStreamSynchronize(ctx->stream));
    for (int i = 0; i < n_pairs; ++i)
        for (int j = 0; j < 9; ++j) F_out_host[(size_t)i * 9 + j] = host[(size_t)i].F[j];
    return LFD_OK;
}

int lfd_upload_cameras(lfd_context* ctx, int32_t n, const float* K, const float* R, const float* t, const float* P,
                       const float* C, const int32_t* wh) {
    if (!ctx) return fail(nullptr, LFD_ERR_INVALID, "null context");
    if (n <= 0 || !K || !R || !t || !P || !C || !wh) return fail(ctx, LFD_ERR_INVALID, "bad camera arrays");
    std::vector<LfdCam> cams((size_t)n);
    for (int i = 0; i < n; ++i) {
        LfdCam& c = cams[i];
        std::memcpy(c.K, K + (size_t)i * 9, sizeof(c.K));
        std::memcpy(c.R, R + (size_t)i * 9, sizeof(c.R));
        std::memcpy(c.t, t + (size_t)i * 3, sizeof(c.t));
        std::memcpy(c.P, P + (size_t)i * 12, sizeof(c.P));
        std::memcpy(c.C, C + (size_t)i * 3, sizeof(c.C));
        c.w = wh[i * 2 + 0]; c.h = wh[i * 2 + 1];
        c.pad[0] = c.pad[1] = 0;
        if (c.w <= 0 || c.h <= 0) return fail(ctx, LFD_ERR_INVALID, "camera width/height must be positive");
    }
    if (ctx->is_host) { ctx->host_cams.swap(cams); ctx->n_cams = n; return LFD_OK; }
    LFD_HIP(ctx, hipSetDevice(ctx->device));
    int rc = ensure(ctx, ctx->cams, cams.size() * sizeof(LfdCam));
    if (rc != LFD_OK) return rc;
    LFD_HIP(ctx, hipMemcpyAsync(ctx->cams.ptr, cams.data(), cams.size() * sizeof(LfdCam), hipMemcpyHostToDevice, ctx->stream));
    LFD_HIP(ctx, hipStreamSynchronize(ctx->stream));
    if (ctx->prep_stream) LFD_HIP(ctx, hipStreamSynchronize(ctx->prep_stream));
    ctx->host_cams.swap(cams);
    ctx->n_cams = n;
    for (LfdBatchSlot& sl : ctx->slot) sl.consts_valid = false;
    return LFD_OK;
}

int lfd_prepare_batch(lfd_context* ctx, const lfd_batch* batch, const lfd_params* params) {
    LfdLaunch L;
    return prepare_launch(ctx, batch, params, nullptr, 0, L, nullptr, true);
}

int lfd_aggregate(lfd_context* ctx, const lfd_batch* batch, const lfd_params* params, float* best_cert, uint8_t* best_slot) {
    LfdLaunch L;
    int rc = prepare_launch(ctx, batch, params, nullptr, 0, L, nullptr);
    if (rc != LFD_OK) return rc;
    if (!best_cert) return fail(ctx, LFD_ERR_INVALID, "best_cert is null");
    const long long HW = (long long)batch->H * batch->W;
    const int per_block = 256 * 4;
    int gx = (int)std::min<long long>((HW + per_block - 1) / per_block, 2048);
    dim3 grid((unsigned)gx, (unsigned)batch->n_refs, 1);
    hipLaunchKernelGGL(lfd_aggregate_kernel, grid, dim3(256), 0, ctx->stream, L, best_cert, best_slot);
    LFD_HIP(ctx, hipGetLastError());
    return LFD_OK;
}

static int dense_launch(lfd_context* ctx, const lfd_batch* batch, const lfd_params* params, const lfd_points* out,
                        int64_t* ref_offsets, int32_t* seg_counts, int64_t* ref_counts, lfd_tile_segment* table, uint8_t* ply = nullptr) {
    const bool unordered = table != nullptr;
    LfdLaunch L;
    int rc = prepare_launch(ctx, batch, params, nullptr, 0, L, nullptr);
    if (rc != LFD_OK) return rc;
    if (ply) {
        if (!out || out->capacity < 0 || !(unordered ? (void*)ref_counts : (void*)ref_offsets))
            return fail(ctx, LFD_ERR_INVALID, "lfd_triangulate_dense_ply[_segments]: the capacity and ref_offsets (ordered) / ref_counts (unordered) are required");
    } else {
        rc = check_points(ctx, out, reinterpret_cast<long long*>(unordered ? ref_counts : ref_offsets));
        if (rc != LFD_OK) return rc;
    }
    if (unordered && out->capacity < (int64_t)batch->n_refs * batch->H * batch->W)
        return fail(ctx, LFD_ERR_CAPACITY, "lfd_triangulate_dense_segments: capacity must be n_refs * H * W (every reference owns a region of H * W records)");
    const size_t n_tiles = (size_t)batch->n_refs * (size_t)L.tiles_per_ref;
    if (n_tiles > 0x7fffffffu) return fail(ctx, LFD_ERR_INVALID, "too many tiles in one launch");
    const size_t grid = n_tiles;
    rc = prepare_lookback(ctx, n_tiles, grid, true, L);
    if (rc != LFD_OK) return rc;
    L.xyz = out->xyz; L.rgb = out->rgb; L.err = out->err; L.cell = out->cell; L.slot = out->slot;
    L.capacity = out->capacity;
    L.ref_offsets = reinterpret_cast<long long*>(ref_offsets);
    L.seg_counts = seg_counts;
    static_assert(sizeof(lfd_tile_segment) == sizeof(LfdTileSeg), "lfd_tile_segment is the kernels' LfdTileSeg");
    L.ref_cursor = reinterpret_cast<unsigned long long*>(ref_counts);
    L.tile_table = reinterpret_cast<LfdTileSeg*>(table);
    L.ply = ply;
    size_t extra_lds = 0;
    extra_lds = ctx->env.dense_extra_lds;
#if defined(LFD_DENSE_TIMING)
    const char* stamp_path = ctx->env.dense_timing_path.empty() ? nullptr : ctx->env.dense_timing_path.c_str();
    if (stamp_path) {
        rc = ensure(ctx, ctx->stamps, n_tiles * 2 * 12 * sizeof(unsigned long long));
        if (rc != LFD_OK) return rc;
        LFD_HIP(ctx, hipMemsetAsync(ctx->stamps.ptr, 0, n_tiles * 2 * 12 * sizeof(unsigned long long), ctx->stream));
        L.phase_stamps = static_cast<unsigned long long*>(ctx->stamps.ptr);
    }
#endif
#if defined(LFD_FORCE_EXACT_COLOUR)
    const bool exact_colour = true;
#else
    const bool exact_colour = (params->flags & LFD_FLAG_EXACT_COLOUR) != 0;
#endif
    if (!exact_colour && L.axis_identity && batch->warp_channels == 2) {
        rc = colour_tables(ctx, batch->W, batch->H, batch->w_match, batch->h_match, &L.colour_cols, &L.colour_rows);
        if (rc != LFD_OK) return rc;
    }
    LfdBatchSlot& used_slot = ctx->slot[ctx->cur];
    rc = slot_events(ctx, used_slot);
    if (rc != LFD_OK) return rc;
    hipEvent_t t_start = nullptr, t_stop = used_slot.idle;
    if (ctx->kt_used < ctx->kt_start.size()) { t_start = ctx->kt_start[ctx->kt_used]; t_stop = ctx->kt_stop[ctx->kt_used]; ++ctx->kt_used; }
    auto kernel = (ply && unordered) ? (exact_colour ? lfd_dense_ply_segments_exact_kernel : lfd_dense_ply_segments_kernel)
                : ply ? (exact_colour ? lfd_dense_ply_exact_kernel : lfd_dense_ply_kernel)
                : unordered ? (exact_colour ? lfd_dense_segments_exact_kernel : lfd_dense_segments_kernel)
                            : (exact_colour ? lfd_dense_exact_kernel : lfd_dense_kernel);
    hipExtLaunchKernelGGL(kernel, dim3((unsigned)grid), dim3(LFD_DENSE_BLOCK), (unsigned)extra_lds, ctx->stream, t_start, t_stop, 0, L);
    LFD_HIP(ctx, hipGetLastError());
    used_slot.idle_ext = t_stop;
    used_slot.idle_attached = true;
#if defined(LFD_DENSE_TIMING)
    if (stamp_path) {
        std::vector<unsigned long long> host(n_tiles * 2 * 12);
        LFD_HIP(ctx, hipMemcpyAsync(host.data(), ctx->stamps.ptr, host.size() * sizeof(unsigned long long), hipMemcpyDeviceToHost, ctx->stream));
        LFD_HIP(ctx, hipStreamSynchronize(ctx->stream));
        if (FILE* f = std::fopen(stamp_path, "wb")) { std::fwrite(host.data(), sizeof(unsigned long long), host.size(), f); std::fclose(f); }
    }
#endif
    return LFD_OK;
}

int lfd_triangulate_dense(lfd_context* ctx, const lfd_batch* batch, const lfd_params* params, const lfd_points* out,
                          int64_t* ref_offsets, int32_t* seg_counts) {
    return dense_launch(ctx, batch, params, out, ref_offsets, seg_counts, nullptr, nullptr);
}

int lfd_triangulate_dense_ply(lfd_context* ctx, const lfd_batch* batch, const lfd_params* params, uint8_t* records, int64_t capacity,
                              int64_t* ref_offsets, int32_t* seg_counts, int32_t* cell, uint8_t* slot) {
    if (ctx && !records) return fail(ctx, LFD_ERR_INVALID, "lfd_triangulate_dense_ply: records is null");
    lfd_points out;
    std::memset(&out, 0, sizeof(out));
    out.capacity = capacity;
    out.cell = cell;
    out.slot = slot;
    return dense_launch(ctx, batch, params, &out, ref_offsets, seg_counts, nullptr, nullptr, records);
}

int lfd_dense_tiles_per_ref(int32_t H, int32_t W) {
    if (H <= 0 || W <= 0) return 0;
    const long long tile = LFD_DENSE_BLOCK * LFD_DENSE_CPT;
    return (int)(((long long)H * W + tile - 1) / tile);
}

int lfd_triangulate_dense_segments(lfd_context* ctx, const lfd_batch* batch, const lfd_params* params, const lfd_points* out,
                                   int64_t* ref_counts, int32_t* seg_counts, lfd_tile_segment* table) {
    if (ctx && !table) return fail(ctx, LFD_ERR_INVALID, "lfd_triangulate_dense_segments: the tile table is required");
    return dense_launch(ctx, batch, params, out, nullptr, seg_counts, ref_counts, table);
}

int lfd_triangulate_dense_ply_segments(lfd_context* ctx, const lfd_batch* batch, const lfd_params* params, uint8_t* records, int64_t capacity,
                                       int64_t* ref_counts, int32_t* seg_counts, lfd_tile_segment* table) {
    if (ctx && (!records || !table)) return fail(ctx, LFD_ERR_INVALID, "lfd_triangulate_dense_ply_segments: records and the tile table are required");
    lfd_points out;
    std::memset(&out, 0, sizeof(out));
    out.capacity = capacity;
    return dense_launch(ctx, batch, params, &out, nullptr, seg_counts, ref_counts, table, records);
}

static int segment_scan(lfd_context* ctx, int32_t n_refs, int32_t H, int32_t W, const lfd_tile_segment* table, int64_t* ref_offsets,
                        const long long** tile_dst, int* tpr_out, int* n_tiles_out) {
    if (!ctx) return fail(nullptr, LFD_ERR_INVALID, "null context");
    if (ctx->is_host) return fail(ctx, LFD_ERR_STATE, "device entry point called on a host context");
    if (n_refs <= 0 || H <= 0 || W <= 0 || !table) return fail(ctx, LFD_ERR_INVALID, "bad segment arguments");
    const int tpr = lfd_dense_tiles_per_ref(H, W);
    const long long n_tiles = (long long)n_refs * tpr;
    if (n_tiles > 0x7fffffffLL) return fail(ctx, LFD_ERR_INVALID, "too many tiles");
    LFD_HIP(ctx, hipSetDevice(ctx->device));
    int rc = ensure(ctx, ctx->seg_scan, ((size_t)n_tiles + 1) * sizeof(long long) + ((size_t)n_tiles + 2) * sizeof(int));
    if (rc != LFD_OK) return rc;
    long long* dst = static_cast<long long*>(ctx->seg_scan.ptr);
    hipLaunchKernelGGL(lfd_segment_scan_kernel, dim3(1), dim3(1024), 0, ctx->stream, reinterpret_cast<const LfdTileSeg*>(table), (int)n_tiles, tpr,
                       (int)n_refs, dst, reinterpret_cast<long long*>(ref_offsets));
    LFD_HIP(ctx, hipGetLastError());
    *tile_dst = dst; *tpr_out = tpr; *n_tiles_out = (int)n_tiles;
    return LFD_OK;
}

int lfd_order_segments(lfd_context* ctx, int32_t n_refs, int32_t H, int32_t W, const lfd_tile_segment* table, const lfd_points* src,
                       const lfd_points* dst, int64_t* ref_offsets) {
    const long long* tile_dst = nullptr; int tpr = 0, n_tiles = 0;
    int rc = segment_scan(ctx, n_refs, H, W, table, ref_offsets, &tile_dst, &tpr, &n_tiles);
    if (rc != LFD_OK) return rc;
    if (!src || !dst || !src->xyz || !src->rgb || !src->err || !dst->xyz || !dst->rgb || !dst->err) return fail(ctx, LFD_ERR_INVALID, "null point buffers");
    if (dst->capacity <= 0) return LFD_OK;
    const unsigned grid = (unsigned)std::min<int64_t>((dst->capacity + 1023) / 1024, 8192);
    hipLaunchKernelGGL(lfd_order_segments_kernel, dim3(grid), dim3(256), 0, ctx->stream, tile_dst, reinterpret_cast<const LfdTileSeg*>(table),
// ... 1526 lines not shown
```

### lichtfeld-densification-plugin_amd/csrc/lfd_context.hpp

```cpp
#pragma once

#include <hip/hip_runtime.h>

#include <string>
#include <vector>

#include "../../include/lfd_densify.h"
#include "lfd_device.hpp"

struct DeviceBuffer {
    void* ptr = nullptr;
    size_t bytes = 0;
};

struct LfdHostPool;
void lfd_host_pool_destroy(LfdHostPool* p);

struct LfdBatchSlot {
    DeviceBuffer desc, consts;
    std::vector<unsigned char> cache;
    bool consts_valid = false;
    int wm = 0, hm = 0, refs = 0, k = 0;
    void* pinned = nullptr;
    size_t pinned_bytes = 0;
    hipEvent_t pinned_free = nullptr;
    bool pinned_in_flight = false;
    void* pinned_x = nullptr;
    size_t pinned_x_bytes = 0;
    hipEvent_t x_free = nullptr;
    bool x_in_flight = false;
    hipEvent_t ready = nullptr;
    bool ready_pending = false;
    hipEvent_t idle = nullptr;
    hipEvent_t idle_ext = nullptr;
    bool idle_attached = false;
    bool used = false;
};

struct LfdEnvSwitches {
    size_t dense_extra_lds = 0;
    std::string dense_timing_path;
    bool indexed_split = true;
    int select_timing = 0;
    int select_workgroups = -1;
};

struct lfd_context {
    LfdEnvSwitches env;
    bool is_host = false;
    int host_threads = 1;
    LfdHostPool* host_pool = nullptr;
    std::vector<unsigned char> host_stage;
    std::vector<LfdCam> host_cams;
    int device = 0;
    hipStream_t stream = nullptr;
    std::string err;
    DeviceBuffer cams;
    int32_t n_cams = 0;
    LfdBatchSlot slot[2];
    int cur = 0;
    int last_used = -1;
    hipStream_t prep_stream = nullptr;
    int* pinned_words = nullptr;
    DeviceBuffer ws;
    unsigned long long tickets_issued = 0;
    unsigned long long lane_issued[LFD_TICKET_LANES] = {};
    unsigned epoch = 0;
    int n_cus = 0;
    DeviceBuffer axes;
    int axes_w = 0, axes_h = 0;
    DeviceBuffer colour_tab;
    int colour_key[4] = {0, 0, 0, 0};
    DeviceBuffer scratch, codes, idx_tab, agg, sel_buf;
    DeviceBuffer mt, sel_scratch, mt_batch;
    DeviceBuffer mt_ckpt;
    unsigned mt_ckpt_taken = 0;
    DeviceBuffer sel_chain;
    DeviceBuffer stamps;
    DeviceBuffer seg_scan;
    DeviceBuffer cloud_ws;
    DeviceBuffer support_ws;
    DeviceBuffer undist_cnt;
    struct PointerTable {
        DeviceBuffer tab;
        std::vector<unsigned char> cache;
        void* pinned = nullptr;
        size_t pinned_bytes = 0;
        hipEvent_t free_ev = nullptr;
        bool in_flight = false;
    };
    PointerTable prec, colour_img;
    PointerTable pose_const;
    DeviceBuffer img_tab, msk_tab;
    int img_key[4] = {0, 0, 0, 0}, img_ks[2] = {0, 0};
    int msk_key[4] = {0, 0, 0, 0}, msk_inv = 0;
    float msk_thr = -1.0f;
    std::vector<hipEvent_t> kt_start, kt_stop;
    size_t kt_used = 0;
    bool mt_seeded = false;
    bool topm_lds_attr_set = false;
};

int lfd_fail(lfd_context* ctx, int code, const std::string& msg);
```

### lichtfeld-densification-plugin_amd/csrc/lfd_geometry.hpp

```cpp
#pragma once

#include <math.h>
#include <stdint.h>

#if defined(__HIPCC__)
#define LFD_HD __host__ __device__ __forceinline__
#else
#define LFD_HD inline
#endif
#if defined(__HIP_DEVICE_COMPILE__)
#define LFD_REREAD_CONSTANTS() asm volatile("" ::: "memory")
#define LFD_OPAQUE4(a, b, c, d) asm volatile("" : "+v"(a), "+v"(b), "+v"(c), "+v"(d) :: "memory")
#else
#define LFD_REREAD_CONSTANTS() do { } while (0)
#define LFD_OPAQUE4(a, b, c, d) do { } while (0)
#endif

struct LfdCam {
    float K[9];
    float R[9];
    float t[3];
    float P[12];
    float C[3];
    int32_t w, h;
// ... 356 lines not shown
    }
    LFD_NULLVEC_SHIFTED_PASSES(LFD_BUILD_M)
    c[0] = x0; c[1] = x1; c[2] = x2; c[3] = x3;
    return it;
#undef LFD_BUILD_M
}

struct LfdCopyRows {
    const float* A;
    LFD_HD void operator()(float* Af) const { for (int i = 0; i < 16; ++i) Af[i] = A[i]; }
};
LFD_HD int lfd_null_vector(const float* Af, double* c) {
    LfdCopyRows rows{Af};
    return lfd_null_vector_rows(rows, c);
}

LFD_HD double lfd_div_by_recip(double a, double b, double r) {
    const double q = a * r;
    return fma(fma(-b, q, a), r, q);
}

LFD_HD float lfd_match_px(float n, float size_m1) {
    return ((n + 1.0f) * 0.5f) * size_m1;
}

LFD_HD float lfd_div_by_recip_f32(float a, float b, float r) {
    const float q = a * r;
    return fmaf(fmaf(-b, q, a), r, q);
}

LFD_HD float lfd_proj_row(const float* Pi, int row, float X0, float X1, float X2, float X3) {
    if (row == 2) return fmaf(X3, Pi[11], fmaf(X2, Pi[10], fmaf(X1, Pi[9], X0 * Pi[8])));
    return fmaf(X3, Pi[6 + row], fmaf(X2, Pi[4 + row], fmaf(X1, Pi[2 + row], X0 * Pi[row])));
}

LFD_HD float lfd_rcp_f32(float x) {
#if defined(__HIP_DEVICE_COMPILE__) && !defined(LFD_IEEE_FINISH)
    return __builtin_amdgcn_rcpf(x);
#else
    return 1.0f / x;
#endif
}
LFD_HD float lfd_sqrt_f32(float x) {
#if defined(__HIP_DEVICE_COMPILE__) && !defined(LFD_IEEE_FINISH)
    return __builtin_amdgcn_sqrtf(x);
#else
    return sqrtf(x);
#endif
}

LFD_HD float lfd_sqrt_rn_f32(float x) {
#if defined(__HIP_DEVICE_COMPILE__)
    const float s = __builtin_amdgcn_sqrtf(x);
    const float h = 0.5f * __builtin_amdgcn_rcpf(s);
    const float r = fmaf(-s, s, x);
    const float c = fmaf(r, h, s);
    return (x > 0.0f && x < 3.0e38f) ? c : s;
#else
    return sqrtf(x);
#endif
}
LFD_HD float lfd_rcp_rn_f32(float b) {
#if defined(__HIP_DEVICE_COMPILE__)
    const float y = __builtin_amdgcn_rcpf(b);
    return fmaf(fmaf(-b, y, 1.0f), y, y);
#else
    return 1.0f / b;
#endif
}

LFD_HD float lfd_reproj_sq(const float* P, float X0, float X1, float X2, float X3, float u, float v, float& pz) {
    const float px = lfd_proj_row(P, 0, X0, X1, X2, X3);
    const float py = lfd_proj_row(P, 1, X0, X1, X2, X3);
    pz = lfd_proj_row(P, 2, X0, X1, X2, X3);
    const float z = fmaxf(pz, 1e-12f);
    const float rz = lfd_rcp_f32(z);
    const float du = lfd_div_by_recip_f32(px, z, rz) - u;
    const float dv = lfd_div_by_recip_f32(py, z, rz) - v;
    return du * du + dv * dv;
}

LFD_HD bool lfd_finite(float x) { return fabsf(x) <= 3.402823466e+38f; }

LFD_HD void lfd_eval_correspondence(const LfdRefConst& rc, const LfdPairConst& pc, float xan, float yan,
                                    float xbn, float ybn, const LfdKernelParams& kp, LfdCellResult& o) {
    const float xa = lfd_match_px(xan, kp.wm1), ya = lfd_match_px(yan, kp.hm1);
    const float xb = lfd_match_px(xbn, kp.wm1), yb = lfd_match_px(ybn, kp.hm1);
    const float ua = xa * rc.sx, va = ya * rc.sy;
    const float ub = xb * pc.sx, vb = yb * pc.sy;
    o.xa_px = xa; o.ya_px = ya;
    o.x = o.y = o.z = 0.0f; o.err = 0.0f; o.keep = 0;

    if (kp.use_sampson) {
        const double x1 = (double)ua, y1 = (double)va, x2 = (double)ub, y2 = (double)vb;
        const double* F = pc.F;
        const double fx0 = fma(F[1], y1, fma(F[0], x1, F[2]));
        const double fx1 = fma(F[4], y1, fma(F[3], x1, F[5]));
        const double fx2 = fma(F[7], y1, fma(F[6], x1, F[8]));
        const double ft0 = fma(F[3], y2, fma(F[0], x2, F[6]));
        const double ft1 = fma(F[4], y2, fma(F[1], x2, F[7]));
        const double num = fma(x2, fx0, fma(y2, fx1, fx2));
        const double den = fma(ft1, ft1, fma(ft0, ft0, fma(fx1, fx1, fx0 * fx0))) + 1e-12;
        if (!((num * num) < kp.sampson_thresh * den)) return;
    }

    struct Rows {
        const LfdRefConst& rc; const LfdPairConst& pc; float ua, va, ub, vb;
        LFD_HD void operator()(float* A) const {
            float u1 = ua, v1 = va, u2 = ub, v2 = vb;
            LFD_OPAQUE4(u1, v1, u2, v2);
#if LFD_PACK_ROWS
            typedef float v2f __attribute__((ext_vector_type(2)));
            const v2f uv1 = {u1, v1}, uv2 = {u2, v2};
#endif
            for (int c = 0; c < 4; ++c) {
#if LFD_PACK_ROWS & 1
                const v2f p1 = {rc.P[2 * c], rc.P[2 * c + 1]};
                const v2f m1 = uv1 * rc.P[8 + c];
                const v2f r1 = m1 - p1;
                A[0 + c] = r1.x; A[4 + c] = r1.y;
#else
                A[0 + c] = u1 * rc.P[8 + c] - rc.P[2 * c];
                A[4 + c] = v1 * rc.P[8 + c] - rc.P[2 * c + 1];
#endif
#if LFD_PACK_ROWS & 2
                const v2f p2 = {pc.P[2 * c], pc.P[2 * c + 1]};
                const v2f m2 = uv2 * pc.P[8 + c];
                const v2f r2 = m2 - p2;
                A[8 + c] = r2.x; A[12 + c] = r2.y;
#else
                A[8 + c] = u2 * pc.P[8 + c] - pc.P[2 * c];
                A[12 + c] = v2 * pc.P[8 + c] - pc.P[2 * c + 1];
#endif
            }
        }
    };
    double c[4];
#if defined(LFD_ABLATE_SOLVER)
    c[0] = ua; c[1] = va; c[2] = ub; c[3] = vb;
#else
    {
        const Rows rows{rc, pc, ua, va, ub, vb};
        lfd_null_vector_rows(rows, c);
    }
#endif
    const double c33 = c[3] * c[3];
    const double n2 = fma(c[0], c[0], fma(c[1], c[1], fma(c[2], c[2], c33)));
    float X0, X1, X2, X3;
    if (c33 < 1e-24 * n2) {
        const double inv = lfd_recip_refined(lfd_sqrt_rare(n2) * 1e-12);
        X0 = (float)(c[0] * inv); X1 = (float)(c[1] * inv); X2 = (float)(c[2] * inv); X3 = (float)(c[3] * inv);
    } else {
        const double r = lfd_recip_refined(c[3]);
        X0 = (float)(c[0] * r);
        X1 = (float)(c[1] * r);
        X2 = (float)(c[2] * r);
        X3 = 1.0f;
    }

    LFD_REREAD_CONSTANTS();
    float z1, z2;
    const float q1 = lfd_reproj_sq(rc.P, X0, X1, X2, X3, ua, va, z1);
    const float q2 = lfd_reproj_sq(pc.P, X0, X1, X2, X3, ub, vb, z2);
    const float qm = (q1 > q2 || q1 != q1) ? q1 : q2;
    const float err = lfd_sqrt_f32(qm);
    o.x = X0; o.y = X1; o.z = X2; o.err = err;

    if (kp.no_filter) {
        o.keep = (lfd_finite(X0) && lfd_finite(X1) && lfd_finite(X2) && lfd_finite(X3) && lfd_finite(err)) ? 1 : 0;
        return;
    }
    bool keep = (err <= kp.reproj_thresh) && (z1 > 0.0f) && (z2 > 0.0f);
    if (keep && kp.use_parallax) {
        const float a0 = X0 - rc.C[0], a1 = X1 - rc.C[1], a2 = X2 - rc.C[2];
        const float b0 = X0 - pc.C[0], b1 = X1 - pc.C[1], b2 = X2 - pc.C[2];
#if LFD_PARALLAX_EXACT
#if LFD_PARALLAX_EXACT >= 3 && defined(__HIP_DEVICE_COMPILE__)
        const float ss_a = (a0 * a0 + a1 * a1) + a2 * a2, ss_b = (b0 * b0 + b1 * b1) + b2 * b2;
#if LFD_PARALLAX_EXACT == 4
        const float nn = lfd_sqrt_f32(ss_a) * lfd_sqrt_f32(ss_b);
        const float dotc = (a0 * b0 + a1 * b1) + a2 * b2;
        const float rhs = kp.dot_thresh * nn, slack = 2e-6f * nn;
        const bool sure_keep = (dotc < rhs - slack) && (nn > 1e-6f), sure_drop = (dotc > rhs + slack) && (nn > 1e-6f);
        if (sure_keep || sure_drop) {
            keep = sure_keep;
        } else
#endif
        {
        const float na = lfd_sqrt_rn_f32(ss_a) + 1e-12f;
        const float nb = lfd_sqrt_rn_f32(ss_b) + 1e-12f;
        const float ra = lfd_rcp_rn_f32(na), rb = lfd_rcp_rn_f32(nb);
        const float ua0 = lfd_div_by_recip_f32(a0, na, ra), ua1 = lfd_div_by_recip_f32(a1, na, ra), ua2 = lfd_div_by_recip_f32(a2, na, ra);
        const float ub0 = lfd_div_by_recip_f32(b0, nb, rb), ub1 = lfd_div_by_recip_f32(b1, nb, rb), ub2 = lfd_div_by_recip_f32(b2, nb, rb);
        const float dot = (ua0 * ub0 + ua1 * ub1) + ua2 * ub2;
        keep = dot <= kp.dot_thresh;
        }
#else
        const float na = sqrtf((a0 * a0 + a1 * a1) + a2 * a2) + 1e-12f;
        const float nb = sqrtf((b0 * b0 + b1 * b1) + b2 * b2) + 1e-12f;
#if LFD_PARALLAX_EXACT == 2 || !defined(__HIP_DEVICE_COMPILE__)
        const float ua0 = a0 / na, ua1 = a1 / na, ua2 = a2 / na;
        const float ub0 = b0 / nb, ub1 = b1 / nb, ub2 = b2 / nb;
#else
        const float ra = 1.0f / na, rb = 1.0f / nb;
        const float ua0 = lfd_div_by_recip_f32(a0, na, ra), ua1 = lfd_div_by_recip_f32(a1, na, ra), ua2 = lfd_div_by_recip_f32(a2, na, ra);
        const float ub0 = lfd_div_by_recip_f32(b0, nb, rb), ub1 = lfd_div_by_recip_f32(b1, nb, rb), ub2 = lfd_div_by_recip_f32(b2, nb, rb);
#endif
        const float dot = (ua0 * ub0 + ua1 * ub1) + ua2 * ub2;
        keep = dot <= kp.dot_thresh;
#endif
#else
        const float na = lfd_sqrt_f32((a0 * a0 + a1 * a1) + a2 * a2) + 1e-12f;
        const float nb = lfd_sqrt_f32((b0 * b0 + b1 * b1) + b2 * b2) + 1e-12f;
        const float dot = (a0 * b0 + a1 * b1) + a2 * b2;
        keep = dot <= kp.dot_thresh * (na * nb);
#endif
    }
    o.keep = keep ? 1 : 0;
}

LFD_HD int lfd_floor_to_i32(float x) {
    const float f = floorf(x);
    if (!(f >= -2147483648.0f && f < 2147483648.0f)) return (int)0x80000000;
    return (int)f;
}

LFD_HD int lfd_clampi(int v, int lo, int hi) { return v < lo ? lo : (v > hi ? hi : v); }

LFD_HD void lfd_bilinear_rgb(const uint8_t* img, int wi, int hi, float xa_px, float ya_px, float sx_img,
                             float sy_img, float* rgb) {
    const float xi = xa_px * sx_img, yi = ya_px * sy_img;
    const int x0 = (int)fminf(fmaxf(floorf(xi), 0.0f), (float)(wi - 1));
    const int y0 = (int)fminf(fmaxf(floorf(yi), 0.0f), (float)(hi - 1));
    const int x1 = lfd_clampi(x0 + 1, 0, wi - 1);
    const int y1 = lfd_clampi(y0 + 1, 0, hi - 1);
    const double xd = (double)xi, yd = (double)yi;
    const double ax = (double)x1 - xd, bx = xd - (double)x0;
    const double ay = (double)y1 - yd, by = yd - (double)y0;
    const double wa = ax * ay, wb = bx * ay, wc = ax * by, wd = bx * by;
    const uint8_t* pa = img + ((unsigned)y0 * (unsigned)wi + (unsigned)x0) * 3u;
    const uint8_t* pb = img + ((unsigned)y0 * (unsigned)wi + (unsigned)x1) * 3u;
    const uint8_t* pcx = img + ((unsigned)y1 * (unsigned)wi + (unsigned)x0) * 3u;
    const uint8_t* pd = img + ((unsigned)y1 * (unsigned)wi + (unsigned)x1) * 3u;
    for (int c = 0; c < 3; ++c) {
        const double s = (((double)(float)pa[c] * wa + (double)(float)pb[c] * wb) + (double)(float)pcx[c] * wc) +
                         (double)(float)pd[c] * wd;
        rgb[c] = (float)lfd_div_by_recip(s, 255.0, 1.0 / 255.0);
    }
}

LFD_HD void lfd_blend4_weights_f32(const float* a, const float* b, const float* c, const float* d, float ax, float bx, float ay, float by,
                                   bool clamped, float* rgb) {
    float wa = ax * ay, wb = bx * ay, wc = ax * by, wd = bx * by;
    if (clamped) {
        wa = wa + wb; wb = 0.0f;
        wc = wc + wd; wd = 0.0f;
    }
    for (int ch = 0; ch < 3; ++ch) {
        const float s = fmaf(d[ch], wd, fmaf(c[ch], wc, fmaf(b[ch], wb, a[ch] * wa)));
        rgb[ch] = s * 0.00392156862745098f;
    }
}

LFD_HD void lfd_blend4_f32(const float* a, const float* b, const float* c, const float* d, int wi, int hi, float xa_px,
                           float ya_px, float* rgb) {
    const float x0 = fminf(fmaxf(floorf(xa_px), 0.0f), (float)(wi - 1));
    const float y0 = fminf(fmaxf(floorf(ya_px), 0.0f), (float)(hi - 1));
    const float x1 = fminf(x0 + 1.0f, (float)(wi - 1));
    const float y1 = fminf(y0 + 1.0f, (float)(hi - 1));
    lfd_blend4_weights_f32(a, b, c, d, x1 - xa_px, xa_px - x0, y1 - ya_px, ya_px - y0, x1 == x0, rgb);
}

struct LfdColourCol { uint32_t off; float ax, bx; uint32_t clamped; };
struct LfdColourRow { uint32_t off0, off1; float ay, by; };
LFD_HD LfdColourCol lfd_colour_col(float xa_px, int wi) {
    const float x0 = fminf(fmaxf(floorf(xa_px), 0.0f), (float)(wi - 1));
    const float x1 = fminf(x0 + 1.0f, (float)(wi - 1));
    LfdColourCol c;
    c.off = 3u * (uint32_t)(int)x0; c.ax = x1 - xa_px; c.bx = xa_px - x0; c.clamped = (x1 == x0) ? 1u : 0u;
    if (x1 == x0) { c.ax = 0.0f; c.bx = 0.0f; }
    return c;
}
LFD_HD LfdColourRow lfd_colour_row(float ya_px, int wi, int hi) {
    const float y0 = fminf(fmaxf(floorf(ya_px), 0.0f), (float)(hi - 1));
    const int iy0 = (int)y0;
    int iy1 = iy0 + 1; if (iy1 > hi - 1) iy1 = hi - 1; if (iy1 < 0) iy1 = 0;
    const float y1 = fminf(y0 + 1.0f, (float)(hi - 1));
    LfdColourRow r;
    r.off0 = 3u * (uint32_t)wi * (uint32_t)iy0; r.off1 = 3u * (uint32_t)wi * (uint32_t)iy1; r.ay = y1 - ya_px; r.by = ya_px - y0;
    return r;
}

LFD_HD void lfd_bilinear_rgb_f32(const uint8_t* img, int wi, int hi, float xa_px, float ya_px, float* rgb) {
    const int x0 = (int)fminf(fmaxf(floorf(xa_px), 0.0f), (float)(wi - 1));
    const int y0 = (int)fminf(fmaxf(floorf(ya_px), 0.0f), (float)(hi - 1));
    const int x1 = lfd_clampi(x0 + 1, 0, wi - 1);
    const int y1 = lfd_clampi(y0 + 1, 0, hi - 1);
    const uint8_t* pa = img + ((size_t)y0 * (size_t)wi + (size_t)x0) * 3u;
    const uint8_t* pb = img + ((size_t)y0 * (size_t)wi + (size_t)x1) * 3u;
    const uint8_t* pc = img + ((size_t)y1 * (size_t)wi + (size_t)x0) * 3u;
    const uint8_t* pd = img + ((size_t)y1 * (size_t)wi + (size_t)x1) * 3u;
// ... 103 lines not shown
```

### lichtfeld-densification-plugin_amd/csrc/lfd_kernels.hip

```cpp
#include <hip/hip_runtime.h>
#include <stdint.h>

#include "lfd_device.hpp"

namespace {

constexpr int kBlock = LFD_DENSE_BLOCK;
constexpr int kCpt = LFD_DENSE_CPT;
constexpr int kTile = kBlock * kCpt;

typedef unsigned long long u64;

constexpr u64 kStEmpty = 0ull, kStAggregate = 1ull, kStPrefix = 2ull;
constexpr u64 kValueMask = (1ull << LFD_VALUE_BITS) - 1ull;
__device__ __forceinline__ u64 pack_state(u64 st, unsigned epoch, u64 v) {
    return (st << 62) | ((u64)epoch << LFD_VALUE_BITS) | (v & kValueMask);
}
__device__ __forceinline__ u64 state_status(u64 s, unsigned epoch) {
    return (((s >> LFD_VALUE_BITS) & LFD_EPOCH_MASK) == epoch) ? (s >> 62) : kStEmpty;
}

__device__ __forceinline__ void state_store(u64* p, u64 v) {
    __hip_atomic_store(p, v, __ATOMIC_RELAXED, __HIP_MEMORY_SCOPE_AGENT);
}
// ... 313 lines not shown
                                                                       uint8_t* __restrict__ best_slot) {
    __shared__ BlockShared S;
    const int r = (int)blockIdx.y;
    const int tid = (int)threadIdx.x;
    if (tid == 0) S.ref = L.refs[r];
    if (tid < L.k) S.slot[tid] = L.slots[(size_t)r * L.k + tid];
    __syncthreads();
    const int HW = L.H * L.W;
    const bool plain = !S.ref.mask_a && (HW & 3) == 0;
    bool any_mask_b = false;
    for (int j = 0; j < S.ref.n_slots; ++j) any_mask_b |= (S.slot[j].mask_b != nullptr);
    const int ns = S.ref.n_slots;
    for (int base = ((int)blockIdx.x * 256 + tid) * 4; base < HW; base += (int)gridDim.x * 256 * 4) {
        if (plain && !any_mask_b && base + 3 < HW) {
            float4 best = load_f32x4(S.slot[0].cert + base);
            const float th = L.kp.certainty_thresh;
            best.x = lfd_cert_floor(best.x, th); best.y = lfd_cert_floor(best.y, th);
            best.z = lfd_cert_floor(best.z, th); best.w = lfd_cert_floor(best.w, th);
            int b0 = 0, b1 = 0, b2 = 0, b3 = 0;
            for (int j = 1; j < ns; ++j) {
                const float4 c = load_f32x4(S.slot[j].cert + base);
                argmax_step(lfd_cert_floor(c.x, th), j, best.x, b0);
                argmax_step(lfd_cert_floor(c.y, th), j, best.y, b1);
                argmax_step(lfd_cert_floor(c.z, th), j, best.z, b2);
                argmax_step(lfd_cert_floor(c.w, th), j, best.w, b3);
            }
            *reinterpret_cast<float4*>(best_cert + (size_t)r * HW + base) = best;
            if (best_slot) {
                const unsigned packed = (unsigned)b0 | ((unsigned)b1 << 8) | ((unsigned)b2 << 16) | ((unsigned)b3 << 24);
                *reinterpret_cast<unsigned*>(best_slot + (size_t)r * HW + base) = packed;
            }
        } else if ((L.W & 3) == 0 && (HW & 3) == 0 && base + 3 < HW) {
            int y, x0;
            lfd_divmod(base, L.W, L.inv_w, y, x0);
            float b4[4]; int j4[4];
            cells4_best_masked(L, S, base, y, x0, b4, j4);
            *reinterpret_cast<float4*>(best_cert + (size_t)r * HW + base) = make_float4(b4[0], b4[1], b4[2], b4[3]);
            if (best_slot) {
                const unsigned packed = (unsigned)j4[0] | ((unsigned)j4[1] << 8) | ((unsigned)j4[2] << 16) | ((unsigned)j4[3] << 24);
                *reinterpret_cast<unsigned*>(best_slot + (size_t)r * HW + base) = packed;
            }
        } else {
            for (int e = 0; e < 4 && base + e < HW; ++e) {
                float best; int bj;
                cell_best(L, S, base + e, best, bj);
                best_cert[(size_t)r * HW + base + e] = best;
                if (best_slot) best_slot[(size_t)r * HW + base + e] = (uint8_t)bj;
            }
        }
    }
}

#define LFD_CONST_AS __attribute__((address_space(4)))
template <class T>
__device__ __forceinline__ const T LFD_CONST_AS* lfd_const_as(const T* p) {
#pragma clang diagnostic push
#pragma clang diagnostic ignored "-Wold-style-cast"
    return (const T LFD_CONST_AS*)p;
#pragma clang diagnostic pop
}

__device__ __forceinline__ int lfd_slot_bytes12(int sl) {
    int o;
    asm("v_mul_u32_u24 %0, %1, 12" : "=v"(o) : "v"(sl));
    return o;
}

struct DenseStage {
    float xyz[3 * kTile];
    float err[kTile];
    unsigned char slot[kTile];
};

struct __attribute__((packed, aligned(4))) LfdF3 { float a, b, c; };

constexpr int kCopyThreadsOrdered = kBlock - 64;

#if defined(LFD_DENSE_TIMING)
#define LFD_STAMP(i) do { if (L.phase_stamps && lane == 0 && wave < 2) L.phase_stamps[((size_t)blockIdx.x * 2 + wave) * 12 + (i)] = __builtin_readcyclecounter(); } while (0)
#else
#define LFD_STAMP(i) do { } while (0)
#endif

template <bool kExactColour, bool kUnordered = false, bool kPly = false>
__device__ __forceinline__ void lfd_dense_body(const LfdLaunch& L) {
    struct DenseShared {
        BlockShared S;
        DenseStage stage;
        u64 tile_excl;
        unsigned ticket;
        unsigned wave_cnt[kBlock / 64];
        unsigned slot_cnt[LFD_MAX_SLOTS];
    };
    __shared__ DenseShared sh;
    BlockShared& S = sh.S;
    DenseStage& stage = sh.stage;
    static_assert(sizeof(sh.S.pc) >= kTile * sizeof(unsigned short), "the order map does not fit the per-pair constant block");
    unsigned short* const stage_order = reinterpret_cast<unsigned short*>(sh.S.pc);
    unsigned& s_ticket = sh.ticket;
    unsigned (&s_wave_cnt)[kBlock / 64] = sh.wave_cnt;
    unsigned (&s_slot_cnt)[LFD_MAX_SLOTS] = sh.slot_cnt;
    u64& s_tile_excl = sh.tile_excl;

    const int tid = (int)threadIdx.x;
    const int lane = tid & 63, wave = tid >> 6;
#if defined(LFD_DENSE_TIMING)
#endif
    LFD_STAMP(0);
    const unsigned seq = blockIdx.x % LFD_TICKET_LANES;
    const unsigned n_tiles = (unsigned)L.n_refs * (unsigned)L.tiles_per_ref;
    const int HW = L.H * L.W;

#if LFD_STAGGER_UNITS > 0
    if (blockIdx.x < (unsigned)LFD_DENSE_WAVES_PER_SIMD * 256u) {
        const unsigned slot = blockIdx.x >> 8;
        for (unsigned i = 0; i < slot; ++i) __builtin_amdgcn_s_sleep(LFD_STAGGER_UNITS);
    }
#endif
    const unsigned tile_guess = blockIdx.x;
    const int r_guess = __builtin_amdgcn_readfirstlane((int)(tile_guess / (unsigned)L.tiles_per_ref));
#if LFD_FRONT_PRIO > 0
    __builtin_amdgcn_s_setprio(LFD_FRONT_PRIO);
#endif
    PrologueRegs pro;
    if (tile_guess < n_tiles) prologue_issue(L, r_guess, pro);
    if (tid == 0) {
        const unsigned long long k = atomicAdd(L.ticket_lanes + (size_t)seq * 16, 1ull) - L.ticket_base_lane[seq];
        s_ticket = (unsigned)k * LFD_TICKET_LANES + seq;
    }
    if (tid < LFD_MAX_SLOTS) s_slot_cnt[tid] = 0;
    if (tile_guess < n_tiles) prologue_commit(L, pro, S);
    __syncthreads();
    LFD_STAMP(1);
    const unsigned tile = s_ticket;
    if (tile == 0 && (L.seg_counts || kUnordered)) {
        if (L.seg_counts) for (int i = tid; i < L.n_refs * L.k; i += kBlock) L.seg_counts[i] = 0;
        if (kUnordered) for (int i = tid; i < L.n_refs; i += kBlock) L.ref_cursor[i] = 0ull;
        __threadfence();
        __syncthreads();
        if (tid == 0) __hip_atomic_store(L.seg_ready, L.epoch, __ATOMIC_RELEASE, __HIP_MEMORY_SCOPE_AGENT);
    }
    if (tile < n_tiles) {
        const int r = __builtin_amdgcn_readfirstlane((int)(tile / (unsigned)L.tiles_per_ref));
        const int tile_in_ref = (int)(tile - (unsigned)r * (unsigned)L.tiles_per_ref);
        LfdRefConst rc;
        {
            const LfdRefConst LFD_CONST_AS* rcp = lfd_const_as(L.ref_const) + r;
#pragma unroll
            for (int i = 0; i < 12; ++i) rc.P[i] = rcp->P[i];
#pragma unroll
            for (int i = 0; i < 3; ++i) rc.C[i] = rcp->C[i];
            rc.sx = rcp->sx; rc.sy = rcp->sy; rc.pad = 0.0f;
        }
        if (r != r_guess || tile_guess >= n_tiles) {
            __syncthreads();
            block_prologue(L, r, S);
        }
        LFD_STAMP(2);
#if defined(LFD_DENSE_TIMING)
        if (L.phase_stamps && lane == 0 && wave < 2) {
            unsigned long long* s0 = L.phase_stamps + ((size_t)blockIdx.x * 2 + wave) * 12;
            *s0 = (*s0 & ~3ull) | (r == r_guess ? 1ull : 0ull) | (tile == tile_guess ? 2ull : 0ull);
        }
#endif
        const int ns = S.ref.n_slots;
        const bool any_mask = S.ref.any_mask != 0;
        const int tile_cell0 = tile_in_ref * kTile;
        const int cell0 = tile_cell0 + tid * kCpt;
        int tile_y0, tile_x0;
        {
            int ty, tx;
            lfd_divmod(tile_cell0, L.W, L.inv_w, ty, tx);
            tile_y0 = __builtin_amdgcn_readfirstlane(ty); tile_x0 = __builtin_amdgcn_readfirstlane(tx);
        }

        int bj[kCpt];
        unsigned dead = 0;
#if LFD_DENSE_ALL_WARPS
        float spec_xb[4] = {0.0f, 0.0f, 0.0f, 0.0f}, spec_yb[4] = {0.0f, 0.0f, 0.0f, 0.0f};
        bool have_warps = false;
        if (!any_mask && (HW & 3) == 0 && kCpt == 4 && cell0 + 3 < HW && ns <= LFD_DENSE_ALL_WARPS && L.warp_channels == 2) {
            const float th = L.kp.certainty_thresh;
            float4 c[4], wa[4], wb[4];
#pragma unroll
            for (int j = 0; j < 4; ++j) {
                if (j < ns) {
                    c[j] = load_f32x4(S.slot[j].cert + cell0);
                    wa[j] = load_f32x4(S.slot[j].warp + (size_t)(unsigned)cell0 * 2);
                    wb[j] = load_f32x4(S.slot[j].warp + (size_t)(unsigned)cell0 * 2 + 4);
                }
            }
            float4 best = c[0];
            best.x = lfd_cert_floor(best.x, th); best.y = lfd_cert_floor(best.y, th);
            best.z = lfd_cert_floor(best.z, th); best.w = lfd_cert_floor(best.w, th);
            bj[0] = bj[1] = bj[2] = bj[3] = 0;
            spec_xb[0] = wa[0].x; spec_yb[0] = wa[0].y; spec_xb[1] = wa[0].z; spec_yb[1] = wa[0].w;
            spec_xb[2] = wb[0].x; spec_yb[2] = wb[0].y; spec_xb[3] = wb[0].z; spec_yb[3] = wb[0].w;
#pragma unroll
            for (int j = 1; j < 4; ++j) {
                if (j < ns) {
                    int t;
                    t = bj[0]; argmax_step(lfd_cert_floor(c[j].x, th), j, best.x, bj[0]); if (bj[0] != t) { spec_xb[0] = wa[j].x; spec_yb[0] = wa[j].y; }
                    t = bj[1]; argmax_step(lfd_cert_floor(c[j].y, th), j, best.y, bj[1]); if (bj[1] != t) { spec_xb[1] = wa[j].z; spec_yb[1] = wa[j].w; }
                    t = bj[2]; argmax_step(lfd_cert_floor(c[j].z, th), j, best.z, bj[2]); if (bj[2] != t) { spec_xb[2] = wb[j].x; spec_yb[2] = wb[j].y; }
                    t = bj[3]; argmax_step(lfd_cert_floor(c[j].w, th), j, best.w, bj[3]); if (bj[3] != t) { spec_xb[3] = wb[j].z; spec_yb[3] = wb[j].w; }
                }
            }
            have_warps = true;
            if (!(th > 0.0f))
                dead = (unsigned)(best.x <= 0.0f) | ((unsigned)(best.y <= 0.0f) << 1) | ((unsigned)(best.z <= 0.0f) << 2) | ((unsigned)(best.w <= 0.0f) << 3);
        } else
#endif
        if (!any_mask && (HW & 3) == 0 && kCpt == 4 && cell0 + 3 < HW) {
            const float th = L.kp.certainty_thresh;
            float4 best;
            bj[0] = bj[1] = bj[2] = bj[3] = 0;
            {
                best = load_f32x4(S.slot[0].cert + cell0);
                best.x = lfd_cert_floor(best.x, th); best.y = lfd_cert_floor(best.y, th);
                best.z = lfd_cert_floor(best.z, th); best.w = lfd_cert_floor(best.w, th);
                for (int j0 = 1; j0 < ns; j0 += 4) {
                    float4 c[4];
#pragma unroll
                    for (int u = 0; u < 4; ++u)
                        if (j0 + u < ns) c[u] = load_f32x4(S.slot[j0 + u].cert + cell0);
#pragma unroll
                    for (int u = 0; u < 4; ++u) {
                        if (j0 + u < ns) {
                            argmax_step(lfd_cert_floor(c[u].x, th), j0 + u, best.x, bj[0]);
                            argmax_step(lfd_cert_floor(c[u].y, th), j0 + u, best.y, bj[1]);
                            argmax_step(lfd_cert_floor(c[u].z, th), j0 + u, best.z, bj[2]);
                            argmax_step(lfd_cert_floor(c[u].w, th), j0 + u, best.w, bj[3]);
                        }
                    }
                }
            }
            if (!(th > 0.0f))
                dead = (unsigned)(best.x <= 0.0f) | ((unsigned)(best.y <= 0.0f) << 1) | ((unsigned)(best.z <= 0.0f) << 2) | ((unsigned)(best.w <= 0.0f) << 3);
        } else if ((L.W & 3) == 0 && (HW & 3) == 0 && kCpt == 4 && cell0 + 3 < HW) {
            int dy, x0;
            lfd_divmod_local(tile_x0 + tid * kCpt, L.W, L.inv_w, L.w_log2, dy, x0);
            float b4[4];
            cells4_best_masked(L, S, cell0, tile_y0 + dy, x0, b4, bj);
#pragma unroll
            for (int e = 0; e < 4; ++e) dead |= (unsigned)(b4[e] <= 0.0f) << e;
        } else {
#pragma unroll
            for (int e = 0; e < kCpt; ++e) {
                bj[e] = 0;
                if (cell0 + e < HW) { float b; cell_best(L, S, cell0 + e, b, bj[e]); dead |= (unsigned)(b <= 0.0f) << e; }
            }
        }

        LFD_STAMP(3);
        unsigned bj_packed = 0;
#if LFD_WARP_BY_LANE
        const bool wave_whole = kCpt == 4 && (L.W & 3) == 0 && tile_cell0 + (wave + 1) * 64 * kCpt <= HW;
#if LFD_DENSE_ALL_WARPS
        const bool by_lane = wave_whole && !have_warps;
#else
        const bool by_lane = wave_whole;
#endif
        if (by_lane) {
            int t2 = (int)threadIdx.x;
            asm volatile("" : "+v"(t2));
            const int ln = t2 & 63, wv = t2 >> 6;
#pragma unroll
            for (int e = 0; e < 4; ++e) bj_packed |= (unsigned)bj[e] << (8 * e);
            *reinterpret_cast<unsigned*>(&stage.slot[t2 * kCpt]) = bj_packed;
            if (L.warp_channels != 4) {
                int dy, x0;
                lfd_divmod_local(tile_x0 + t2 * kCpt, L.W, L.inv_w, L.w_log2, dy, x0);
                const int y0 = tile_y0 + dy;
                float xa[4], ya;
                if (L.axis_identity) {
#pragma unroll
                    for (int e = 0; e < 4; ++e) xa[e] = lfd_axis_value(L.ax, x0 + e);
                    ya = lfd_axis_value(L.ay, y0);
                } else {
                    const float4 ax = load_f32x4(L.axis_x + x0);
                    xa[0] = ax.x; xa[1] = ax.y; xa[2] = ax.z; xa[3] = ax.w;
                    ya = lfd_global(L.axis_y)[y0];
                }
#pragma unroll
                for (int e = 0; e < 4; ++e) { stage.xyz[3 * (t2 * kCpt + e) + 0] = xa[e]; stage.xyz[3 * (t2 * kCpt + e) + 1] = ya; }
            }
            __builtin_amdgcn_fence(__ATOMIC_ACQ_REL, "wavefront");
            __builtin_amdgcn_wave_barrier();
            const int wbase = wv * 64 * kCpt + ln;
            int sj[4];
#pragma unroll
            for (int e = 0; e < 4; ++e) sj[e] = (int)stage.slot[wbase + 64 * e];
            if (L.warp_channels == 4) {
                float4 v[4];
#pragma unroll
                for (int e = 0; e < 4; ++e) v[e] = load_f32x4(S.slot[sj[e]].warp + (size_t)(unsigned)(tile_cell0 + wbase + 64 * e) * 4);
#pragma unroll
                for (int e = 0; e < 4; ++e) {
                    const int sl = wbase + 64 * e;
                    stage.xyz[3 * sl + 0] = v[e].x; stage.xyz[3 * sl + 1] = v[e].y; stage.xyz[3 * sl + 2] = v[e].z;
                    stage.err[sl] = v[e].w;
                }
            } else {
                float2 v[4];
#pragma unroll
                for (int e = 0; e < 4; ++e) v[e] = load_f32x2(S.slot[sj[e]].warp + (size_t)(unsigned)(tile_cell0 + wbase + 64 * e) * 2);
#pragma unroll
                for (int e = 0; e < 4; ++e) {
                    const int sl = wbase + 64 * e;
                    stage.xyz[3 * sl + 2] = v[e].x;
                    stage.err[sl] = v[e].y;
                }
            }
            __builtin_amdgcn_fence(__ATOMIC_ACQ_REL, "wavefront");
            __builtin_amdgcn_wave_barrier();
        } else
#endif
        if (kCpt == 4 && (L.W & 3) == 0 && cell0 + 3 < HW) {
            float xa[4] = {0.0f, 0.0f, 0.0f, 0.0f}, ya = 0.0f;
            if (L.warp_channels != 4) {
                int dy, x0;
                lfd_divmod_local(tile_x0 + tid * kCpt, L.W, L.inv_w, L.w_log2, dy, x0);
                const int y0 = tile_y0 + dy;
                if (L.axis_identity) {
#pragma unroll
                    for (int e = 0; e < 4; ++e) xa[e] = lfd_axis_value(L.ax, x0 + e);
                    ya = lfd_axis_value(L.ay, y0);
                } else {
                    const float4 ax = load_f32x4(L.axis_x + x0);
                    xa[0] = ax.x; xa[1] = ax.y; xa[2] = ax.z; xa[3] = ax.w;
                    ya = lfd_global(L.axis_y)[y0];
                }
            }
#pragma unroll
            for (int e = 0; e < 4; ++e) {
                const float* wp = S.slot[bj[e]].warp;
                float xan, yan, xbn, ybn;
                if (L.warp_channels == 4) {
                    const float4 v = load_f32x4(wp + (size_t)(unsigned)(cell0 + e) * 4);
                    xan = v.x; yan = v.y; xbn = v.z; ybn = v.w;
#if LFD_DENSE_ALL_WARPS
                } else if (have_warps) {
                    xan = xa[e]; yan = ya; xbn = spec_xb[e]; ybn = spec_yb[e];
#endif
                } else {
                    const float2 v = load_f32x2(wp + (size_t)(unsigned)(cell0 + e) * 2);
                    xan = xa[e]; yan = ya; xbn = v.x; ybn = v.y;
                }
                const int sl = tid * kCpt + e;
                stage.xyz[3 * sl + 0] = xan; stage.xyz[3 * sl + 1] = yan; stage.xyz[3 * sl + 2] = xbn;
                stage.err[sl] = ybn;
                bj_packed |= (unsigned)bj[e] << (8 * e);
            }
        } else {
#pragma unroll
            for (int e = 0; e < kCpt; ++e) {
                float xan = 0.0f, yan = 0.0f, xbn = 0.0f, ybn = 0.0f;
                if (cell0 + e < HW) cell_coords(L, S, cell0 + e, bj[e], xan, yan, xbn, ybn);
                const int sl = tid * kCpt + e;
                stage.xyz[3 * sl + 0] = xan; stage.xyz[3 * sl + 1] = yan; stage.xyz[3 * sl + 2] = xbn;
                stage.err[sl] = ybn;
                bj_packed |= (unsigned)bj[e] << (8 * e);
            }
        }
        if (dead) {
#pragma unroll
            for (int e = 0; e < kCpt; ++e)
                if ((dead >> e) & 1u) stage.xyz[3 * (tid * kCpt + e) + 2] = __builtin_nanf("");
        }
        *reinterpret_cast<unsigned*>(&stage.slot[tid * kCpt]) = bj_packed;

        LFD_STAMP(4);
#if LFD_FRONT_PRIO > 0
        __builtin_amdgcn_s_setprio(0);
#endif
        unsigned keep_bits = 0;
#pragma unroll 1
        for (int ev = 0; ev < kCpt; ++ev) {
            asm volatile("" ::: "memory");
            const int e = __builtin_amdgcn_readfirstlane(ev);
            const int sl = tid * kCpt + e;
            float* sxyz = reinterpret_cast<float*>(reinterpret_cast<unsigned char*>(stage.xyz) + lfd_slot_bytes12(sl));
            const float xan = sxyz[0], yan = sxyz[1], xbn = sxyz[2];
            const float ybn = stage.err[sl];
            const int bje = (int)((bj_packed >> (8 * e)) & 0xffu);
            LfdCellResult res;
            res.keep = 0; res.x = res.y = res.z = res.err = res.xa_px = res.ya_px = 0.0f;
#if defined(LFD_ABLATE_EVAL)
            if (cell0 + e < HW) { res.keep = xbn > -0.9f; res.x = xan; res.y = yan; res.z = xbn; res.err = ybn; res.xa_px = 1.0f; res.ya_px = 1.0f; }
#else
            if (cell0 + e < HW) lfd_eval_correspondence(rc, S.pc[bje], xan, yan, xbn, ybn, L.kp, res);
#endif
            if (res.keep) {
                sxyz[0] = res.x; sxyz[1] = res.y; sxyz[2] = res.z;
                stage.err[sl] = res.err;
                keep_bits |= 1u << e;
            }
        }
        LFD_STAMP(5);
#if defined(LFD_BACK_PRIO)
        __builtin_amdgcn_s_setprio(LFD_BACK_PRIO);
#endif
        if (L.seg_counts) {
            for (int j = 0; j < ns; ++j) {
                unsigned c = 0;
#pragma unroll
                for (int e = 0; e < kCpt; ++e)
                    c += (unsigned)__popcll(__ballot(((keep_bits >> e) & 1u) && ((bj_packed >> (8 * e)) & 0xffu) == (unsigned)j));
                if (lane == 0 && c) atomicAdd(&s_slot_cnt[j], c);
            }
        }

        const unsigned my_cnt = __popc(keep_bits);
        unsigned before = 0, wave_total = 0;
#pragma unroll
        for (int e = 0; e < kCpt; ++e) {
            const u64 m = __ballot((keep_bits >> e) & 1u);
            before += __builtin_amdgcn_mbcnt_hi((unsigned)(m >> 32), __builtin_amdgcn_mbcnt_lo((unsigned)m, 0u));
            wave_total += (unsigned)__popcll(m);
        }
        const unsigned incl = before + my_cnt;
        if (lane == 0) s_wave_cnt[wave] = wave_total;
        __syncthreads();
        LFD_STAMP(6);
        unsigned wave_off = 0, block_total = 0;
#pragma unroll
        for (int w = 0; w < kBlock / 64; ++w) {
            if (w < wave) wave_off += s_wave_cnt[w];
            block_total += s_wave_cnt[w];
        }
        {
            unsigned lpos = wave_off + (incl - my_cnt);
#pragma unroll
            for (int e = 0; e < kCpt; ++e)
                if ((keep_bits >> e) & 1u) stage_order[lpos++] = (unsigned short)(tid * kCpt + e);
        }
        __syncthreads();
        LFD_STAMP(7);
        if (L.seg_counts && tid < ns && s_slot_cnt[tid]) {
            unsigned spins = 0;
            unsigned ready = __hip_atomic_load(L.seg_ready, __ATOMIC_RELAXED, __HIP_MEMORY_SCOPE_AGENT);
            while (ready != L.epoch) {
                if (++spins > LFD_SPIN_LIMIT) { atomicExch(L.status, LFD_LAUNCH_TIMEOUT); break; }
                __builtin_amdgcn_s_sleep(8);
                ready = __hip_atomic_load(L.seg_ready, __ATOMIC_RELAXED, __HIP_MEMORY_SCOPE_AGENT);
            }
            atomicAdd(&L.seg_counts[(size_t)r * L.k + tid], (int)s_slot_cnt[tid]);
        }

        constexpr int kCopyThreads = kUnordered ? kBlock : kCopyThreadsOrdered;
        constexpr int kCopyRecords = (kTile + kCopyThreads - 1) / kCopyThreads;
        float rgb[kCopyRecords][3];
        int ctid = (int)threadIdx.x;
        asm volatile("" : "+v"(ctid));
        if (!kUnordered) ctid -= 64;
        u64 claimed = 0;
        if (kUnordered && tid == 0) {
            unsigned spins = 0;
            unsigned ready = __hip_atomic_load(L.seg_ready, __ATOMIC_RELAXED, __HIP_MEMORY_SCOPE_AGENT);
            while (ready != L.epoch) {
                if (++spins > LFD_SPIN_LIMIT) { atomicExch(L.status, LFD_LAUNCH_TIMEOUT); break; }
                __builtin_amdgcn_s_sleep(8);
                ready = __hip_atomic_load(L.seg_ready, __ATOMIC_RELAXED, __HIP_MEMORY_SCOPE_AGENT);
            }
            claimed = atomicAdd(L.ref_cursor + r, (u64)block_total);
        }
        if (!kUnordered && wave == 0) {
#if defined(LFD_ABLATE_LOOKBACK)
            const u64 excl = (u64)tile * kTile;
#else
            const u64 excl = lookback_exclusive(L, tile, block_total);
#endif
            if (lane == 0) {
                s_tile_excl = excl;
                if (tile_in_ref == 0) L.ref_offsets[r] = (long long)excl;
                if (tile == n_tiles - 1u) L.ref_offsets[L.n_refs] = (long long)(excl + block_total);
            }
        }
        if (kUnordered || wave != 0) {
#if !defined(LFD_ABLATE_STORES)
            const uint8_t* image = S.ref.image;
            const int n_loc = (int)block_total;
            if (!kExactColour && L.colour_cols) {
                const unsigned n_bytes = __umul24((unsigned)L.w_match, (unsigned)L.h_match) * 3u;
#pragma unroll
                for (int u0 = 0; u0 < kCopyRecords; u0 += LFD_COPY_UNROLL) {
                    LfdColourCol cc[LFD_COPY_UNROLL];
                    LfdColourRow cr[LFD_COPY_UNROLL];
                    LfdTapRows taps[LFD_COPY_UNROLL];
                    unsigned sh0[LFD_COPY_UNROLL], sh1[LFD_COPY_UNROLL];
                    if (ctid + u0 * kCopyThreads < n_loc) {
#pragma unroll
                        for (int v = 0; v < LFD_COPY_UNROLL; ++v) {
                            if (u0 + v >= kCopyRecords) break;
                            const int i = ctid + (u0 + v) * kCopyThreads;
                            const int sl = (int)stage_order[i < n_loc ? i : n_loc - 1];
                            int dy, x;
                            lfd_divmod_local(tile_x0 + sl, L.W, L.inv_w, L.w_log2, dy, x);
                            const lfd_u32x4 c4 = *reinterpret_cast<const lfd_u32x4 LFD_GLOBAL_AS*>(lfd_global(L.colour_cols) + x);
                            const lfd_u32x4 r4 = *reinterpret_cast<const lfd_u32x4 LFD_GLOBAL_AS*>(lfd_global(L.colour_rows) + (tile_y0 + dy));
                            cc[v].off = c4.x; cc[v].ax = __uint_as_float(c4.y); cc[v].bx = __uint_as_float(c4.z); cc[v].clamped = c4.w;
                            cr[v].off0 = r4.x; cr[v].off1 = r4.y; cr[v].ay = __uint_as_float(r4.z); cr[v].by = __uint_as_float(r4.w);
                            taps[v] = lfd_bilinear_fetch_tab(image, n_bytes, cc[v], cr[v], sh0[v], sh1[v]);
                        }
#pragma unroll
                        for (int v = 0; v < LFD_COPY_UNROLL; ++v) {
                            if (u0 + v >= kCopyRecords) break;
                            lfd_bilinear_eval_tab(taps[v], sh0[v], sh1[v], cc[v], cr[v], rgb[u0 + v]);
                        }
                    }
                }
            } else {
#pragma unroll
            for (int u0 = 0; u0 < kCopyRecords; u0 += LFD_COPY_UNROLL) {
                float px[LFD_COPY_UNROLL], py[LFD_COPY_UNROLL];
                LfdTapRows taps[LFD_COPY_UNROLL];
                unsigned sh0[LFD_COPY_UNROLL], sh1[LFD_COPY_UNROLL];
                if (ctid + u0 * kCopyThreads < n_loc) {
#pragma unroll
                    for (int v = 0; v < LFD_COPY_UNROLL; ++v) {
                        if (u0 + v >= kCopyRecords) break;
                        const int i = ctid + (u0 + v) * kCopyThreads;
                        const int sl = (int)stage_order[i < n_loc ? i : n_loc - 1];
                        {
                            const int cell = tile_cell0 + sl;
                            float xan, yan;
                            if (L.warp_channels == 4) {
                                const float2 w2 = load_f32x2(S.slot[stage.slot[sl]].warp + (size_t)cell * 4);
                                xan = w2.x; yan = w2.y;
                            } else {
                                int dy, x;
                                lfd_divmod_local(tile_x0 + sl, L.W, L.inv_w, L.w_log2, dy, x);
                                const int y = tile_y0 + dy;
                                if (L.axis_identity) { xan = lfd_axis_value(L.ax, x); yan = lfd_axis_value(L.ay, y); }
                                else { xan = lfd_global(L.axis_x)[x]; yan = lfd_global(L.axis_y)[y]; }
                            }
                            px[v] = lfd_match_px(xan, L.kp.wm1); py[v] = lfd_match_px(yan, L.kp.hm1);
                        }
                        taps[v] = lfd_bilinear_fetch(image, L.w_match, L.h_match, px[v], py[v], sh0[v], sh1[v]);
                    }
#pragma unroll
                    for (int v = 0; v < LFD_COPY_UNROLL; ++v) {
                        if (u0 + v >= kCopyRecords) break;
#if defined(LFD_ABLATE_COLOUR)
                        rgb[u0 + v][0] = px[v]; rgb[u0 + v][1] = py[v]; rgb[u0 + v][2] = (float)(taps[v].r0 + taps[v].r1 + sh0[v] + sh1[v]);
#else
                        if (kExactColour) lfd_bilinear_eval(taps[v], sh0[v], sh1[v], L.w_match, L.h_match, px[v], py[v], rgb[u0 + v]);
                        else lfd_bilinear_eval_f32(taps[v], sh0[v], sh1[v], L.w_match, L.h_match, px[v], py[v], rgb[u0 + v]);
#endif
                    }
                }
            }
            }
#endif
        }
        if (kUnordered && tid == 0) {
            s_tile_excl = (u64)(unsigned)r * (u64)(unsigned)HW + claimed;
            LfdTileSeg seg; seg.offset = (int32_t)claimed; seg.count = (int32_t)block_total;
            L.tile_table[tile] = seg;
        }
        LFD_STAMP(8);
        __syncthreads();
        LFD_STAMP(9);

#if !defined(LFD_ABLATE_STORES)
        if (kUnordered || wave != 0) {
            const u64 excl = s_tile_excl;
            const long long base = (long long)(((u64)(unsigned)__builtin_amdgcn_readfirstlane((int)(unsigned)(excl >> 32)) << 32) |
                                               (u64)(unsigned)__builtin_amdgcn_readfirstlane((int)(unsigned)excl));
            long long room = L.capacity - base;
            int n = (int)block_total;
            if (room < (long long)n) n = room > 0 ? (int)room : 0;
            if (kPly) {
                unsigned char* gp = L.ply + 15 * base;
#pragma unroll
                for (int u = 0; u < kCopyRecords; ++u) {
                    const int i = ctid + u * kCopyThreads;
                    if (i < n) {
                        const int sl = (int)stage_order[i];
                        const float* sxyz = reinterpret_cast<const float*>(reinterpret_cast<const unsigned char*>(stage.xyz) + lfd_slot_bytes12(sl));
                        struct __attribute__((packed, aligned(1))) F3u { float a, b, c; };
                        struct __attribute__((packed, aligned(1))) U16u { unsigned short v; };
                        F3u p; p.a = sxyz[0]; p.b = sxyz[1]; p.c = sxyz[2];
                        const unsigned o15 = (unsigned)i * 15u;
                        const unsigned q0 = lfd_quantise_u8(rgb[u][0]), q1 = lfd_quantise_u8(rgb[u][1]), q2 = lfd_quantise_u8(rgb[u][2]);
                        *reinterpret_cast<F3u*>(gp + o15) = p;
                        U16u rg; rg.v = (unsigned short)(q0 | (q1 << 8));
                        *reinterpret_cast<U16u*>(gp + o15 + 12u) = rg;
                        gp[o15 + 14u] = (unsigned char)q2;
                        if (L.cell) L.cell[base + i] = tile_cell0 + sl;
                        if (L.slot) L.slot[base + i] = stage.slot[sl];
                    }
                }
            } else {
            unsigned char* gx = reinterpret_cast<unsigned char*>(L.xyz + 3 * base);
            unsigned char* gc = reinterpret_cast<unsigned char*>(L.rgb + 3 * base);
            unsigned char* ge = reinterpret_cast<unsigned char*>(L.err + base);
#pragma unroll
            for (int u = 0; u < kCopyRecords; ++u) {
                const int i = ctid + u * kCopyThreads;
                if (i < n) {
                    const int sl = (int)stage_order[i];
                    LfdF3 p, c;
                    const float* sxyz = reinterpret_cast<const float*>(reinterpret_cast<const unsigned char*>(stage.xyz) + lfd_slot_bytes12(sl));
                    p.a = sxyz[0]; p.b = sxyz[1]; p.c = sxyz[2];
                    c.a = rgb[u][0]; c.b = rgb[u][1]; c.c = rgb[u][2];
                    const unsigned o12 = (unsigned)lfd_slot_bytes12(i), o4 = (unsigned)i * 4u;
#if LFD_NT_STORES
                    float* fx = reinterpret_cast<float*>(gx + o12);
                    float* fc = reinterpret_cast<float*>(gc + o12);
                    __builtin_nontemporal_store(p.a, fx); __builtin_nontemporal_store(p.b, fx + 1); __builtin_nontemporal_store(p.c, fx + 2);
                    __builtin_nontemporal_store(c.a, fc); __builtin_nontemporal_store(c.b, fc + 1); __builtin_nontemporal_store(c.c, fc + 2);
                    __builtin_nontemporal_store(stage.err[sl], reinterpret_cast<float*>(ge + o4));
#else
                    *reinterpret_cast<LfdF3*>(gx + o12) = p;
                    *reinterpret_cast<LfdF3*>(gc + o12) = c;
                    *reinterpret_cast<float*>(ge + o4) = stage.err[sl];
#endif
                    if (L.cell) L.cell[base + i] = tile_cell0 + sl;
                    if (L.slot) L.slot[base + i] = stage.slot[sl];
                }
            }
        }
#endif
            }
#if defined(LFD_DENSE_TIMING)
        LFD_STAMP(10);
        if (L.phase_stamps && lane == 0 && wave < 2) {
            asm volatile("s_waitcnt vmcnt(0)" ::: "memory");
            L.phase_stamps[((size_t)blockIdx.x * 2 + wave) * 12 + 11] = __builtin_readcyclecounter();
        }
#endif
    }
}

extern "C" __global__ void __launch_bounds__(kBlock, LFD_DENSE_WAVES_PER_SIMD) lfd_dense_kernel(LfdLaunch L) { lfd_dense_body<false>(L); }
extern "C" __global__ void __launch_bounds__(kBlock, LFD_DENSE_WAVES_PER_SIMD) lfd_dense_exact_kernel(LfdLaunch L) { lfd_dense_body<true>(L); }
extern "C" __global__ void __launch_bounds__(kBlock, LFD_DENSE_WAVES_PER_SIMD) lfd_dense_ply_kernel(LfdLaunch L) { lfd_dense_body<false, false, true>(L); }
extern "C" __global__ void __launch_bounds__(kBlock, LFD_DENSE_WAVES_PER_SIMD) lfd_dense_ply_exact_kernel(LfdLaunch L) { lfd_dense_body<true, false, true>(L); }
extern "C" __global__ void __launch_bounds__(kBlock, LFD_DENSE_WAVES_PER_SIMD) lfd_dense_segments_kernel(LfdLaunch L) { lfd_dense_body<false, true>(L); }
extern "C" __global__ void __launch_bounds__(kBlock, LFD_DENSE_WAVES_PER_SIMD) lfd_dense_segments_exact_kernel(LfdLaunch L) { lfd_dense_body<true, true>(L); }
extern "C" __global__ void __launch_bounds__(kBlock, LFD_DENSE_WAVES_PER_SIMD) lfd_dense_ply_segments_kernel(LfdLaunch L) { lfd_dense_body<false, true, true>(L); }
extern "C" __global__ void __launch_bounds__(kBlock, LFD_DENSE_WAVES_PER_SIMD) lfd_dense_ply_segments_exact_kernel(LfdLaunch L) { lfd_dense_body<true, true, true>(L); }

extern "C" __global__ void __launch_bounds__(LFD_INDEXED_EVAL_BLOCK) lfd_indexed_eval_kernel(LfdLaunch L, const long long* __restrict__ sel_idx,
                                                                                             const long long* __restrict__ sel_offsets,
                                                                                             float* __restrict__ scratch, uint8_t* __restrict__ codes,
                                                                                             unsigned* __restrict__ tab, int off_pairs) {
    __shared__ BlockShared S;
    __shared__ unsigned s_cnt[LFD_MAX_SLOTS];
    __shared__ unsigned s_first[LFD_MAX_SLOTS];
    const int tid = (int)threadIdx.x;
    const int r = (int)blockIdx.y;
    const long long sel_begin = off_pairs ? sel_offsets[2 * r] : sel_offsets[r], sel_end = off_pairs ? sel_offsets[2 * r + 1] : sel_offsets[r + 1];
    const int n_sel = (int)(sel_end - sel_begin);
    const int i = (int)blockIdx.x * LFD_INDEXED_EVAL_BLOCK + tid;
    if ((int)blockIdx.x * LFD_INDEXED_EVAL_BLOCK >= n_sel) return;
    if (tid < LFD_MAX_SLOTS) { s_cnt[tid] = 0; s_first[tid] = 0xffffffffu; }
    block_prologue(L, r, S);
    const int HW = L.H * L.W;
    if (i < n_sel) {
        const long long cl = sel_idx[sel_begin + i];
        unsigned code = 0xffu;
        if (cl >= 0 && cl < HW) {
            const int cell = (int)cl;
            float best; int bj;
            cell_best(L, S, cell, best, bj);
            float xan, yan, xbn, ybn;
            cell_coords(L, S, cell, bj, xan, yan, xbn, ybn);
            LfdCellResult res;
            lfd_eval_correspondence(S.rc, S.pc[bj], xan, yan, xbn, ybn, L.kp, res);
            atomicMin(&s_first[bj], (unsigned)i);
            code = (unsigned)bj | (res.keep ? 0x80u : 0u);
            if (res.keep) {
                float rgb[3];
                lfd_bilinear_rgb(S.ref.image, L.w_match, L.h_match, res.xa_px, res.ya_px, 1.0f, 1.0f, rgb);
                float* o = scratch + (size_t)(sel_begin + i) * 8;
                o[0] = res.x; o[1] = res.y; o[2] = res.z; o[3] = res.err; o[4] = rgb[0]; o[5] = rgb[1]; o[6] = rgb[2];
                atomicAdd(&s_cnt[bj], 1u);
            }
        }
        codes[sel_begin + i] = (uint8_t)code;
    }
    __syncthreads();
    if (tid < LFD_MAX_SLOTS) {
        unsigned* t = tab + ((size_t)r * LFD_MAX_SLOTS + tid) * 2;
        if (s_cnt[tid]) atomicAdd(t + 0, s_cnt[tid]);
        if (s_first[tid] != 0xffffffffu) atomicMax(t + 1, 0xffffffffu - s_first[tid]);
    }
}

extern "C" __global__ void __launch_bounds__(LFD_INDEXED_BLOCK) lfd_indexed_kernel(LfdLaunch L, const long long* __restrict__ sel_idx,
                                                                                   const long long* __restrict__ sel_offsets,
                                                                                   float* __restrict__ scratch, uint8_t* __restrict__ codes,
                                                                                   int32_t* __restrict__ seg_order, const unsigned* __restrict__ tab, int off_pairs) {
    __shared__ BlockShared S;
    __shared__ unsigned s_ticket;
    __shared__ unsigned s_cnt[LFD_MAX_SLOTS];
    __shared__ unsigned s_first[LFD_MAX_SLOTS];
    __shared__ unsigned s_start[LFD_MAX_SLOTS];
    __shared__ unsigned s_run[LFD_MAX_SLOTS];
    __shared__ unsigned s_wcnt[LFD_INDEXED_BLOCK / 64][LFD_MAX_SLOTS];
    __shared__ u64 s_excl;
    __shared__ unsigned s_total;

    const int tid = (int)threadIdx.x, lane = tid & 63, wave = tid >> 6;
    constexpr int nwaves = LFD_INDEXED_BLOCK / 64;
    if (tid == 0) s_ticket = (unsigned)(atomicAdd(L.ticket, 1ull) - L.ticket_base);
    if (tid < LFD_MAX_SLOTS) { s_cnt[tid] = 0; s_first[tid] = 0xffffffffu; s_run[tid] = 0; }
    __syncthreads();
    const int r = (int)s_ticket;
    block_prologue(L, r, S);
    const int ns = S.ref.n_slots;
    const long long sel_begin = off_pairs ? sel_offsets[2 * r] : sel_offsets[r], sel_end = off_pairs ? sel_offsets[2 * r + 1] : sel_offsets[r + 1];
    const int n_sel = (int)(sel_end - sel_begin);
    const int HW = L.H * L.W;

    if (tab) {
        if (tid < LFD_MAX_SLOTS) {
            s_cnt[tid] = tab[((size_t)r * LFD_MAX_SLOTS + tid) * 2 + 0];
// ... 94 lines not shown
```

Measured before the change: 52.46 billion.

## Add specialised production-shape dense kernel and order-only events without system fence

```diff
diff --git a/include/lfd_densify.h b/include/lfd_densify.h
--- a/include/lfd_densify.h
+++ b/include/lfd_densify.h
@@ -83,6 +83,8 @@
 int lfd_triangulate_dense(lfd_context* ctx, const lfd_batch* batch, const lfd_params* params,
                           const lfd_points* out, int64_t* ref_offsets, int32_t* seg_counts);
 
+int lfd_dense_variant(const lfd_batch* batch, const lfd_params* params, const lfd_points* out, const int32_t* seg_counts);
+
 int lfd_triangulate_dense_ply(lfd_context* ctx, const lfd_batch* batch, const lfd_params* params, uint8_t* records, int64_t capacity,
                               int64_t* ref_offsets, int32_t* seg_counts, int32_t* cell, uint8_t* slot);
 
diff --git a/lichtfeld-densification-plugin_amd/core/hip_backend.py b/lichtfeld-densification-plugin_amd/core/hip_backend.py
--- a/lichtfeld-densification-plugin_amd/core/hip_backend.py
+++ b/lichtfeld-densification-plugin_amd/core/hip_backend.py
@@ -159,6 +159,8 @@
     lib.lfd_triangulate_dense_ply.argtypes = [ctxp, C.POINTER(lfd_batch), C.POINTER(lfd_params), C.c_void_p, C.c_int64, C.c_void_p, C.c_void_p,
                                               C.c_void_p, C.c_void_p]
     lib.lfd_dense_tiles_per_ref.argtypes = [C.c_int32, C.c_int32]
+    lib.lfd_dense_variant.argtypes = [C.POINTER(lfd_batch), C.POINTER(lfd_params), C.POINTER(lfd_points), C.c_void_p]
+    lib.lfd_dense_variant.restype = C.c_int
     lib.lfd_triangulate_dense_segments.argtypes = [ctxp, C.POINTER(lfd_batch), C.POINTER(lfd_params), C.POINTER(lfd_points),
                                                    C.c_void_p, C.c_void_p, C.c_void_p]
     lib.lfd_triangulate_dense_ply_segments.argtypes = [ctxp, C.POINTER(lfd_batch), C.POINTER(lfd_params), C.c_void_p, C.c_int64, C.c_void_p, C.c_void_p, C.c_void_p]
@@ -313,6 +315,10 @@
                       flags=LFD_FLAG_EXACT_COLOUR if exact_colour else 0)
 
 
+def dense_variant(batch: lfd_batch, params: lfd_params, out: lfd_points, seg_counts: Optional[int] = None) -> int:
+    return int(load_library().lfd_dense_variant(C.byref(batch), C.byref(params), C.byref(out), seg_counts))
+
+
 def _f32(a) -> np.ndarray:
     return np.ascontiguousarray(np.asarray(a, np.float32))
 
diff --git a/lichtfeld-densification-plugin_amd/csrc/lfd_api.hip b/lichtfeld-densification-plugin_amd/csrc/lfd_api.hip
--- a/lichtfeld-densification-plugin_amd/csrc/lfd_api.hip
+++ b/lichtfeld-densification-plugin_amd/csrc/lfd_api.hip
@@ -38,6 +38,7 @@
 extern "C" __global__ void lfd_aggregate_kernel(LfdLaunch L, float* best_cert, uint8_t* best_slot);
 extern "C" __global__ void lfd_dense_kernel(LfdLaunch L);
 extern "C" __global__ void lfd_dense_exact_kernel(LfdLaunch L);
+extern "C" __global__ void lfd_dense_prod_kernel(LfdLaunch L);
 extern "C" __global__ void lfd_dense_ply_kernel(LfdLaunch L);
 extern "C" __global__ void lfd_dense_ply_exact_kernel(LfdLaunch L);
 extern "C" __global__ void lfd_dense_segments_kernel(LfdLaunch L);
@@ -224,10 +225,12 @@
     return LFD_OK;
 }
 
+constexpr unsigned kOrderOnly = hipEventDisableTiming | hipEventDisableSystemFence;
+
 int slot_events(lfd_context* ctx, LfdBatchSlot& sl) {
-    if (!sl.pinned_free) LFD_HIP(ctx, hipEventCreateWithFlags(&sl.pinned_free, hipEventDisableTiming));
-    if (!sl.ready) LFD_HIP(ctx, hipEventCreateWithFlags(&sl.ready, hipEventDisableTiming));
-    if (!sl.idle) LFD_HIP(ctx, hipEventCreateWithFlags(&sl.idle, hipEventDisableTiming));
+    if (!sl.pinned_free) LFD_HIP(ctx, hipEventCreateWithFlags(&sl.pinned_free, kOrderOnly));
+    if (!sl.ready) LFD_HIP(ctx, hipEventCreateWithFlags(&sl.ready, kOrderOnly));
+    if (!sl.idle) LFD_HIP(ctx, hipEventCreateWithFlags(&sl.idle, kOrderOnly));
     return LFD_OK;
 }
 
@@ -322,7 +325,7 @@
             sl.pinned_x_bytes = std::max<size_t>(extra_room * 2, 4096);
             LFD_HIP(ctx, hipHostMalloc(&sl.pinned_x, sl.pinned_x_bytes, hipHostMallocDefault));
         }
-        if (!sl.x_free) LFD_HIP(ctx, hipEventCreateWithFlags(&sl.x_free, hipEventDisableTiming));
+        if (!sl.x_free) LFD_HIP(ctx, hipEventCreateWithFlags(&sl.x_free, kOrderOnly));
         std::memcpy(sl.pinned_x, extra, n_extra * sizeof(long long));
         LFD_HIP(ctx, hipMemcpyAsync(static_cast<unsigned char*>(sl.desc.ptr) + off_extra, sl.pinned_x, n_extra * sizeof(long long), hipMemcpyHostToDevice,
                                     ctx->stream));
@@ -499,6 +502,7 @@
     ctx->env = LfdEnvSwitches();
     if (const char* e = std::getenv("LFD_DENSE_EXTRA_LDS")) ctx->env.dense_extra_lds = (size_t)std::atol(e);
     if (const char* e = std::getenv("LFD_DENSE_TIMING")) ctx->env.dense_timing_path = e;
+    if (const char* e = std::getenv("LFD_DENSE_GENERIC")) ctx->env.dense_generic = std::atoi(e) != 0;
     if (const char* e = std::getenv("LFD_INDEXED_SPLIT")) ctx->env.indexed_split = std::atoi(e) != 0;
     if (const char* e = std::getenv("LFD_SELECT_TIMING")) ctx->env.select_timing = std::max(1, std::atoi(e));
     if (const char* e = std::getenv("LFD_SELECT_WORKGROUPS")) ctx->env.select_workgroups = std::atoi(e);
@@ -757,8 +761,8 @@
     }
     while (ctx->kt_start.size() < (size_t)n_launches) {
         hipEvent_t a = nullptr, b = nullptr;
-        LFD_HIP(ctx, hipEventCreate(&a));
-        hipError_t e = hipEventCreate(&b);
+        LFD_HIP(ctx, hipEventCreateWithFlags(&a, hipEventDisableSystemFence));
+        hipError_t e = hipEventCreateWithFlags(&b, hipEventDisableSystemFence);
         if (e != hipSuccess) { (void)hipEventDestroy(a); return fail(ctx, LFD_ERR_HIP, std::string("hipEventCreate: ") + hipGetErrorString(e)); }
         ctx->kt_start.push_back(a); ctx->kt_stop.push_back(b);
     }
@@ -877,6 +881,26 @@
     hipLaunchKernelGGL(lfd_aggregate_kernel, grid, dim3(256), 0, ctx->stream, L, best_cert, best_slot);
     LFD_HIP(ctx, hipGetLastError());
     return LFD_OK;
+}
+
+int lfd_dense_variant(const lfd_batch* b, const lfd_params* p, const lfd_points* out, const int32_t* seg_counts) {
+    if (!b || !p || !out) return 0;
+    const long long tile = LFD_DENSE_BLOCK * LFD_DENSE_CPT;
+    if (b->n_refs <= 0 || b->H <= 0 || b->W <= 0 || (b->W & 3) != 0 || ((long long)b->H * b->W) % tile != 0) return 0;
+    if (b->warp_channels != 2 || b->axis_x || b->axis_y) return 0;
+    if ((p->flags & LFD_FLAG_EXACT_COLOUR) != 0) return 0;
+    if (!(p->certainty_thresh > 0.0f)) return 0;
+    if (p->no_filter || !(p->sampson_thresh > 0.0) || !(p->min_parallax_deg > 0.0f)) return 0;
+    if (seg_counts || out->cell || out->slot) return 0;
+    if (b->mask_a || b->mask_b) {
+        if (!b->n_slots) return 0;
+        for (int r = 0; r < b->n_refs; ++r) {
+            if (b->mask_a && b->mask_a[r]) return 0;
+            for (int j = 0; b->mask_b && j < b->n_slots[r] && j < b->k; ++j)
+                if (b->mask_b[(size_t)r * b->k + j]) return 0;
+        }
+    }
+    return 1;
 }
 
 static int dense_launch(lfd_context* ctx, const lfd_batch* batch, const lfd_params* params, const lfd_points* out,
@@ -932,7 +956,9 @@
     if (rc != LFD_OK) return rc;
     hipEvent_t t_start = nullptr, t_stop = used_slot.idle;
     if (ctx->kt_used < ctx->kt_start.size()) { t_start = ctx->kt_start[ctx->kt_used]; t_stop = ctx->kt_stop[ctx->kt_used]; ++ctx->kt_used; }
-    auto kernel = (ply && unordered) ? (exact_colour ? lfd_dense_ply_segments_exact_kernel : lfd_dense_ply_segments_kernel)
+    const bool prod = !ply && !unordered && !exact_colour && !ctx->env.dense_generic && L.colour_cols && lfd_dense_variant(batch, params, out, seg_counts) == 1;
+    auto kernel = prod ? lfd_dense_prod_kernel
+                : (ply && unordered) ? (exact_colour ? lfd_dense_ply_segments_exact_kernel : lfd_dense_ply_segments_kernel)
                 : ply ? (exact_colour ? lfd_dense_ply_exact_kernel : lfd_dense_ply_kernel)
                 : unordered ? (exact_colour ? lfd_dense_segments_exact_kernel : lfd_dense_segments_kernel)
                             : (exact_colour ? lfd_dense_exact_kernel : lfd_dense_kernel);
diff --git a/lichtfeld-densification-plugin_amd/csrc/lfd_context.hpp b/lichtfeld-densification-plugin_amd/csrc/lfd_context.hpp
--- a/lichtfeld-densification-plugin_amd/csrc/lfd_context.hpp
+++ b/lichtfeld-densification-plugin_amd/csrc/lfd_context.hpp
@@ -40,6 +40,7 @@
 struct LfdEnvSwitches {
     size_t dense_extra_lds = 0;
     std::string dense_timing_path;
+    bool dense_generic = false;
     bool indexed_split = true;
     int select_timing = 0;
     int select_workgroups = -1;
diff --git a/lichtfeld-densification-plugin_amd/csrc/lfd_geometry.hpp b/lichtfeld-densification-plugin_amd/csrc/lfd_geometry.hpp
--- a/lichtfeld-densification-plugin_amd/csrc/lfd_geometry.hpp
+++ b/lichtfeld-densification-plugin_amd/csrc/lfd_geometry.hpp
@@ -462,8 +462,9 @@
 
 LFD_HD bool lfd_finite(float x) { return fabsf(x) <= 3.402823466e+38f; }
 
-LFD_HD void lfd_eval_correspondence(const LfdRefConst& rc, const LfdPairConst& pc, float xan, float yan,
-                                    float xbn, float ybn, const LfdKernelParams& kp, LfdCellResult& o) {
+template <bool kAllGates>
+LFD_HD void lfd_eval_correspondence_as(const LfdRefConst& rc, const LfdPairConst& pc, float xan, float yan,
+                                       float xbn, float ybn, const LfdKernelParams& kp, LfdCellResult& o) {
     const float xa = lfd_match_px(xan, kp.wm1), ya = lfd_match_px(yan, kp.hm1);
     const float xb = lfd_match_px(xbn, kp.wm1), yb = lfd_match_px(ybn, kp.hm1);
     const float ua = xa * rc.sx, va = ya * rc.sy;
@@ -471,7 +472,7 @@
     o.xa_px = xa; o.ya_px = ya;
     o.x = o.y = o.z = 0.0f; o.err = 0.0f; o.keep = 0;
 
-    if (kp.use_sampson) {
+    if (kAllGates || kp.use_sampson) {
         const double x1 = (double)ua, y1 = (double)va, x2 = (double)ub, y2 = (double)vb;
         const double* F = pc.F;
         const double fx0 = fma(F[1], y1, fma(F[0], x1, F[2]));
@@ -546,12 +547,12 @@
     const float err = lfd_sqrt_f32(qm);
     o.x = X0; o.y = X1; o.z = X2; o.err = err;
 
-    if (kp.no_filter) {
+    if (!kAllGates && kp.no_filter) {
         o.keep = (lfd_finite(X0) && lfd_finite(X1) && lfd_finite(X2) && lfd_finite(X3) && lfd_finite(err)) ? 1 : 0;
         return;
     }
     bool keep = (err <= kp.reproj_thresh) && (z1 > 0.0f) && (z2 > 0.0f);
-    if (keep && kp.use_parallax) {
+    if (keep && (kAllGates || kp.use_parallax)) {
         const float a0 = X0 - rc.C[0], a1 = X1 - rc.C[1], a2 = X2 - rc.C[2];
         const float b0 = X0 - pc.C[0], b1 = X1 - pc.C[1], b2 = X2 - pc.C[2];
 #if LFD_PARALLAX_EXACT
@@ -597,6 +598,11 @@
 #endif
     }
     o.keep = keep ? 1 : 0;
+}
+
+LFD_HD void lfd_eval_correspondence(const LfdRefConst& rc, const LfdPairConst& pc, float xan, float yan,
+                                    float xbn, float ybn, const LfdKernelParams& kp, LfdCellResult& o) {
+    lfd_eval_correspondence_as<false>(rc, pc, xan, yan, xbn, ybn, kp, o);
 }
 
 LFD_HD int lfd_floor_to_i32(float x) {
diff --git a/lichtfeld-densification-plugin_amd/csrc/lfd_kernels.hip b/lichtfeld-densification-plugin_amd/csrc/lfd_kernels.hip
--- a/lichtfeld-densification-plugin_amd/csrc/lfd_kernels.hip
+++ b/lichtfeld-densification-plugin_amd/csrc/lfd_kernels.hip
@@ -419,8 +419,10 @@
 #define LFD_STAMP(i) do { } while (0)
 #endif
 
-template <bool kExactColour, bool kUnordered = false, bool kPly = false>
+template <bool kExactColour, bool kUnordered = false, bool kPly = false, bool kProd = false>
 __device__ __forceinline__ void lfd_dense_body(const LfdLaunch& L) {
+    static_assert(!kProd || (!kExactColour && !kUnordered && !kPly), "the production-shape kernel is the ordered f32-colour one");
+    static_assert(!kProd || (LFD_WARP_BY_LANE && !LFD_DENSE_ALL_WARPS && kCpt == 4), "the production-shape kernel parks by lane (see kProdBuild)");
     struct DenseShared {
         BlockShared S;
         DenseStage stage;
@@ -465,12 +467,12 @@
         const unsigned long long k = atomicAdd(L.ticket_lanes + (size_t)seq * 16, 1ull) - L.ticket_base_lane[seq];
         s_ticket = (unsigned)k * LFD_TICKET_LANES + seq;
     }
-    if (tid < LFD_MAX_SLOTS) s_slot_cnt[tid] = 0;
+    if (!kProd && tid < LFD_MAX_SLOTS) s_slot_cnt[tid] = 0;
     if (tile_guess < n_tiles) prologue_commit(L, pro, S);
     __syncthreads();
     LFD_STAMP(1);
     const unsigned tile = s_ticket;
-    if (tile == 0 && (L.seg_counts || kUnordered)) {
+    if (!kProd && tile == 0 && (L.seg_counts || kUnordered)) {
         if (L.seg_counts) for (int i = tid; i < L.n_refs * L.k; i += kBlock) L.seg_counts[i] = 0;
         if (kUnordered) for (int i = tid; i < L.n_refs; i += kBlock) L.ref_cursor[i] = 0ull;
         __threadfence();
@@ -501,7 +503,7 @@
         }
 #endif
         const int ns = S.ref.n_slots;
-        const bool any_mask = S.ref.any_mask != 0;
+        const bool any_mask = !kProd && S.ref.any_mask != 0;
         const int tile_cell0 = tile_in_ref * kTile;
         const int cell0 = tile_cell0 + tid * kCpt;
         int tile_y0, tile_x0;
@@ -548,7 +550,7 @@
                 dead = (unsigned)(best.x <= 0.0f) | ((unsigned)(best.y <= 0.0f) << 1) | ((unsigned)(best.z <= 0.0f) << 2) | ((unsigned)(best.w <= 0.0f) << 3);
         } else
 #endif
-        if (!any_mask && (HW & 3) == 0 && kCpt == 4 && cell0 + 3 < HW) {
+        if (kProd || (!any_mask && (HW & 3) == 0 && kCpt == 4 && cell0 + 3 < HW)) {
             const float th = L.kp.certainty_thresh;
             float4 best;
             bj[0] = bj[1] = bj[2] = bj[3] = 0;
@@ -572,7 +574,7 @@
                     }
                 }
             }
-            if (!(th > 0.0f))
+            if (!kProd && !(th > 0.0f))
                 dead = (unsigned)(best.x <= 0.0f) | ((unsigned)(best.y <= 0.0f) << 1) | ((unsigned)(best.z <= 0.0f) << 2) | ((unsigned)(best.w <= 0.0f) << 3);
         } else if ((L.W & 3) == 0 && (HW & 3) == 0 && kCpt == 4 && cell0 + 3 < HW) {
             int dy, x0;
@@ -592,7 +594,7 @@
         LFD_STAMP(3);
         unsigned bj_packed = 0;
 #if LFD_WARP_BY_LANE
-        const bool wave_whole = kCpt == 4 && (L.W & 3) == 0 && tile_cell0 + (wave + 1) * 64 * kCpt <= HW;
+        const bool wave_whole = kProd || (kCpt == 4 && (L.W & 3) == 0 && tile_cell0 + (wave + 1) * 64 * kCpt <= HW);
 #if LFD_DENSE_ALL_WARPS
         const bool by_lane = wave_whole && !have_warps;
 #else
@@ -605,12 +607,12 @@
 #pragma unroll
             for (int e = 0; e < 4; ++e) bj_packed |= (unsigned)bj[e] << (8 * e);
             *reinterpret_cast<unsigned*>(&stage.slot[t2 * kCpt]) = bj_packed;
-            if (L.warp_channels != 4) {
+            if (kProd || L.warp_channels != 4) {
                 int dy, x0;
                 lfd_divmod_local(tile_x0 + t2 * kCpt, L.W, L.inv_w, L.w_log2, dy, x0);
                 const int y0 = tile_y0 + dy;
                 float xa[4], ya;
-                if (L.axis_identity) {
+                if (kProd || L.axis_identity) {
 #pragma unroll
                     for (int e = 0; e < 4; ++e) xa[e] = lfd_axis_value(L.ax, x0 + e);
                     ya = lfd_axis_value(L.ay, y0);
@@ -628,7 +630,7 @@
             int sj[4];
 #pragma unroll
             for (int e = 0; e < 4; ++e) sj[e] = (int)stage.slot[wbase + 64 * e];
-            if (L.warp_channels == 4) {
+            if (!kProd && L.warp_channels == 4) {
                 float4 v[4];
 #pragma unroll
                 for (int e = 0; e < 4; ++e) v[e] = load_f32x4(S.slot[sj[e]].warp + (size_t)(unsigned)(tile_cell0 + wbase + 64 * e) * 4);
@@ -653,7 +655,8 @@
             __builtin_amdgcn_wave_barrier();
         } else
 #endif
-        if (kCpt == 4 && (L.W & 3) == 0 && cell0 + 3 < HW) {
+        if (kProd) {
+        } else if (kCpt == 4 && (L.W & 3) == 0 && cell0 + 3 < HW) {
             float xa[4] = {0.0f, 0.0f, 0.0f, 0.0f}, ya = 0.0f;
             if (L.warp_channels != 4) {
                 int dy, x0;
@@ -700,12 +703,12 @@
                 bj_packed |= (unsigned)bj[e] << (8 * e);
             }
         }
-        if (dead) {
+        if (!kProd && dead) {
 #pragma unroll
             for (int e = 0; e < kCpt; ++e)
                 if ((dead >> e) & 1u) stage.xyz[3 * (tid * kCpt + e) + 2] = __builtin_nanf("");
         }
-        *reinterpret_cast<unsigned*>(&stage.slot[tid * kCpt]) = bj_packed;
+        if (!kProd) *reinterpret_cast<unsigned*>(&stage.slot[tid * kCpt]) = bj_packed;
 
         LFD_STAMP(4);
 #if LFD_FRONT_PRIO > 0
@@ -726,7 +729,8 @@
 #if defined(LFD_ABLATE_EVAL)
             if (cell0 + e < HW) { res.keep = xbn > -0.9f; res.x = xan; res.y = yan; res.z = xbn; res.err = ybn; res.xa_px = 1.0f; res.ya_px = 1.0f; }
 #else
-            if (cell0 + e < HW) lfd_eval_correspondence(rc, S.pc[bje], xan, yan, xbn, ybn, L.kp, res);
+            if (kProd) lfd_eval_correspondence_as<true>(rc, S.pc[bje], xan, yan, xbn, ybn, L.kp, res);
+            else if (cell0 + e < HW) lfd_eval_correspondence(rc, S.pc[bje], xan, yan, xbn, ybn, L.kp, res);
 #endif
             if (res.keep) {
                 sxyz[0] = res.x; sxyz[1] = res.y; sxyz[2] = res.z;
@@ -738,7 +742,7 @@
 #if defined(LFD_BACK_PRIO)
         __builtin_amdgcn_s_setprio(LFD_BACK_PRIO);
 #endif
-        if (L.seg_counts) {
+        if (!kProd && L.seg_counts) {
             for (int j = 0; j < ns; ++j) {
                 unsigned c = 0;
 #pragma unroll
@@ -774,7 +778,7 @@
         }
         __syncthreads();
         LFD_STAMP(7);
-        if (L.seg_counts && tid < ns && s_slot_cnt[tid]) {
+        if (!kProd && L.seg_counts && tid < ns && s_slot_cnt[tid]) {
             unsigned spins = 0;
             unsigned ready = __hip_atomic_load(L.seg_ready, __ATOMIC_RELAXED, __HIP_MEMORY_SCOPE_AGENT);
             while (ready != L.epoch) {
@@ -818,7 +822,7 @@
 #if !defined(LFD_ABLATE_STORES)
             const uint8_t* image = S.ref.image;
             const int n_loc = (int)block_total;
-            if (!kExactColour && L.colour_cols) {
+            if (kProd || (!kExactColour && L.colour_cols)) {
                 const unsigned n_bytes = __umul24((unsigned)L.w_match, (unsigned)L.h_match) * 3u;
 #pragma unroll
                 for (int u0 = 0; u0 < kCopyRecords; u0 += LFD_COPY_UNROLL) {
@@ -954,8 +958,8 @@
                     *reinterpret_cast<LfdF3*>(gc + o12) = c;
                     *reinterpret_cast<float*>(ge + o4) = stage.err[sl];
 #endif
-                    if (L.cell) L.cell[base + i] = tile_cell0 + sl;
-                    if (L.slot) L.slot[base + i] = stage.slot[sl];
+                    if (!kProd && L.cell) L.cell[base + i] = tile_cell0 + sl;
+                    if (!kProd && L.slot) L.slot[base + i] = stage.slot[sl];
                 }
             }
         }
@@ -973,6 +977,8 @@
 
 extern "C" __global__ void __launch_bounds__(kBlock, LFD_DENSE_WAVES_PER_SIMD) lfd_dense_kernel(LfdLaunch L) { lfd_dense_body<false>(L); }
 extern "C" __global__ void __launch_bounds__(kBlock, LFD_DENSE_WAVES_PER_SIMD) lfd_dense_exact_kernel(LfdLaunch L) { lfd_dense_body<true>(L); }
+constexpr bool kProdBuild = LFD_WARP_BY_LANE && !LFD_DENSE_ALL_WARPS && kCpt == 4;
+extern "C" __global__ void __launch_bounds__(kBlock, LFD_DENSE_WAVES_PER_SIMD) lfd_dense_prod_kernel(LfdLaunch L) { lfd_dense_body<false, false, false, kProdBuild>(L); }
 extern "C" __global__ void __launch_bounds__(kBlock, LFD_DENSE_WAVES_PER_SIMD) lfd_dense_ply_kernel(LfdLaunch L) { lfd_dense_body<false, false, true>(L); }
 extern "C" __global__ void __launch_bounds__(kBlock, LFD_DENSE_WAVES_PER_SIMD) lfd_dense_ply_exact_kernel(LfdLaunch L) { lfd_dense_body<true, false, true>(L); }
 extern "C" __global__ void __launch_bounds__(kBlock, LFD_DENSE_WAVES_PER_SIMD) lfd_dense_segments_kernel(LfdLaunch L) { lfd_dense_body<false, true>(L); }
```

New measurement: 53.97 billion, median of 6. 1.03x the previous value.
